# pierreaubert/math-audio

Hardware: NVIDIA B200
Metric: bem_assemble_plus_gmres_seconds_per_frequency (lower is better)
Workload: dtype f64

## Files before the change

### include/bemb200.h

```cpp
#ifndef BEMB200_H
#define BEMB200_H

#include <stdint.h>

#ifdef __cplusplus
extern "C" {
#endif

#define BEMB200_OK 0
#define BEMB200_EINVAL (-1)
#define BEMB200_ENODEVICE (-2)
#define BEMB200_ECUDA (-3)
#define BEMB200_ENOMEM (-4)
#define BEMB200_ENCCL (-5)
#define BEMB200_EUNSUPPORTED (-6)
#define BEMB200_ESINGULAR (-7)
#define BEMB200_ECALLBACK (-8)

typedef struct bemb200_ctx bemb200_ctx;
typedef struct bemb200_staged_mesh bemb200_staged_mesh;
typedef struct bemb200_matrix bemb200_matrix;

typedef struct bemb200_mesh {
    uint64_t n_nodes;
    uint64_t n_elem;
    const double* nodes;
    const uint32_t* conn;
    const uint8_t* etype;
    const double* center;
    const double* normal;
    const double* area;
    const int32_t* bc_type;
    const uint8_t* bc_len;
    const double* bc_val;
    const uint32_t* dof;
    const uint8_t* is_eval;
} bemb200_mesh;

typedef struct bemb200_physics {
    double wave_number;
    double harmonic_factor;
    double tau;
    double gamma;
} bemb200_physics;

typedef struct bemb200_gmres_info {
    uint64_t iterations;
    uint64_t restarts;
    double residual;
    int32_t converged;
} bemb200_gmres_info;

typedef struct bemb200_assembly_stats {
    uint64_t near_pairs;
    uint64_t special_pairs;
    uint64_t far_kernel_launches;
    uint64_t total_launches;
    double far_ms;
    double total_ms;
} bemb200_assembly_stats;

int bemb200_device_count(void);
int bemb200_ctx_create(int device, bemb200_ctx** out);
int bemb200_nccl_unique_id(uint8_t out[128]);
int bemb200_ctx_create_dist(int device, int rank, int nranks, const uint8_t nccl_id[128], bemb200_ctx** out);
int bemb200_ctx_create_ex(int device, int rank, int nranks, const uint8_t* nccl_id, void* cuda_stream, bemb200_ctx** out);
void bemb200_ctx_destroy(bemb200_ctx* ctx);
int bemb200_ctx_set_background(bemb200_ctx* ctx, int blocks_per_sm);
int bemb200_ctx_set_shared_gpu(bemb200_ctx* ctx, int shared);
int bemb200_matrix_boost_assembly(bemb200_matrix* m, bemb200_ctx* ctx);
int bemb200_ctx_peer_exchange_active(const bemb200_ctx* ctx, int* active);
int bemb200_matrix_set_context(bemb200_matrix* m, bemb200_ctx* ctx);
const char* bemb200_last_error(const bemb200_ctx* ctx);
void bemb200_partition(uint64_t n, int nranks, int rank, uint64_t* row_begin, uint64_t* row_end);

int bemb200_mesh_stage(bemb200_ctx* ctx, const bemb200_mesh* mesh, bemb200_staged_mesh** out);
void bemb200_staged_mesh_free(bemb200_staged_mesh* sm);
uint64_t bemb200_staged_num_dofs(const bemb200_staged_mesh* sm);
int bemb200_assemble_staged(bemb200_ctx* ctx, const bemb200_staged_mesh* sm, const bemb200_physics* phys, double beta_re,
                            double beta_im, uint64_t row_begin, uint64_t row_end, bemb200_matrix** inout);
int bemb200_assemble(bemb200_ctx* ctx, const bemb200_mesh* mesh, const bemb200_physics* phys, double beta_re,
                     double beta_im, uint64_t row_begin, uint64_t row_end, bemb200_matrix** out);
int bemb200_assembly_stats_get(const bemb200_matrix* m, bemb200_assembly_stats* out);
double bemb200_dg_dn_sign(const bemb200_staged_mesh* sm, double wave_number);

int bemb200_matrix_from_host(bemb200_ctx* ctx, const double* a_rows, uint64_t n_rows_global, uint64_t n_cols,
                             uint64_t row_begin, uint64_t row_end, bemb200_matrix** out);
void bemb200_matrix_free(bemb200_matrix* m);
uint64_t bemb200_num_rows(const bemb200_matrix* m);
uint64_t bemb200_num_cols(const bemb200_matrix* m);
uint64_t bemb200_local_row_begin(const bemb200_matrix* m);
uint64_t bemb200_local_row_end(const bemb200_matrix* m);
int bemb200_matrix_download(const bemb200_matrix* m, uint64_t row_begin, uint64_t row_end, double* out);
int bemb200_rhs_download(const bemb200_matrix* m, double* out);
int bemb200_rhs_download_full(const bemb200_matrix* m, double* out);
int bemb200_row_sum_correction(bemb200_matrix* m, double* avg);

int bemb200_apply(const bemb200_matrix* m, const double* x, double* y);
int bemb200_apply_transpose(const bemb200_matrix* m, const double* x, double* y);
int bemb200_apply_device(const bemb200_matrix* m, const double* x_dev, double* y_dev);

int bemb200_gmres(const bemb200_matrix* m, const double* b, const double* x0, uint32_t max_iterations, uint32_t restart,
                  double tolerance, double* x_out, bemb200_gmres_info* info);
int bemb200_gmres_preconditioned(const bemb200_matrix* m, const double* inv_diag, const double* b, const double* x0,
                                 uint32_t max_iterations, uint32_t restart, double tolerance, double* x_out,
                                 bemb200_gmres_info* info);
int bemb200_matrix_diagonal(const bemb200_matrix* m, double* out);
typedef struct bemb200_precond bemb200_precond;
typedef struct bemb200_precond_stats {
    uint32_t num_subdomains;
    uint32_t local_subdomains;
    uint32_t min_size, max_size;
    double avg_size;
    uint64_t inverse_bytes;
    double factor_ms;
    int32_t disjoint;
} bemb200_precond_stats;
int bemb200_schwarz_create(const bemb200_matrix* m, uint32_t num_subdomains, const uint64_t* sub_ptr, const uint64_t* sub_idx,
                           bemb200_precond** out);
void bemb200_precond_free(bemb200_precond* p);
int bemb200_precond_stats_get(const bemb200_precond* p, bemb200_precond_stats* out);
int bemb200_precond_apply(const bemb200_precond* p, const double* r, double* z);
int bemb200_gmres_schwarz(const bemb200_matrix* m, const bemb200_precond* precond, const double* b, const double* x0,
                          uint32_t max_iterations, uint32_t restart, double tolerance, double* x_out, bemb200_gmres_info* info);
typedef int (*bemb200_precond_fn)(void* user, const double* r, double* z, uint64_t n);
int bemb200_gmres_callback(const bemb200_matrix* m, bemb200_precond_fn apply, void* user, const double* b, const double* x0,
                           uint32_t max_iterations, uint32_t restart, double tolerance, double* x_out, bemb200_gmres_info* info,
                           uint64_t* precond_calls);
int bemb200_gmres_device(const bemb200_matrix* m, const double* b_dev, const double* x0_dev, uint32_t max_iterations,
                         uint32_t restart, double tolerance, double* x_dev, bemb200_gmres_info* info);
int bemb200_lu_solve(const bemb200_matrix* m, const double* b, double* x_out, int overwrite_matrix, double* factor_ms);
int bemb200_bicgstab(const bemb200_matrix* m, const double* b, uint32_t max_iterations, double tolerance, double* x_out,
                     bemb200_gmres_info* info);
int bemb200_cgs(const bemb200_matrix* m, const double* b, uint32_t max_iterations, double tolerance, double* x_out,
                bemb200_gmres_info* info);
int bemb200_gmres_batched(const bemb200_matrix* m, const double* b_all, uint32_t nrhs, uint32_t max_iterations,
                          uint32_t restart, double tolerance, double* x_all, bemb200_gmres_info* infos,
                          double* block_matvec_ms, uint64_t* block_matvecs);
int bemb200_gmres_batched_schwarz(const bemb200_matrix* m, const bemb200_precond* precond, const double* b_all, uint32_t nrhs,
                                  uint32_t max_iterations, uint32_t restart, double tolerance, double* x_all,
                                  bemb200_gmres_info* infos, double* block_matvec_ms, uint64_t* block_matvecs);
int bemb200_apply_block(const bemb200_matrix* m, const double* x_all, uint32_t nrhs, double* y_all, double* kernel_ms);
int bemb200_solver_stats(const bemb200_matrix* m, uint64_t* kernel_launches, double* matvec_ms, uint64_t* matvecs);

int bemb200_incident_rhs(const bemb200_staged_mesh* sm, const bemb200_physics* phys, double beta_re, double beta_im,
                         uint32_t n_sources, const int32_t* kinds, const double* vecs, const double* amps, double* rhs_host,
                         double* rhs_dev);
int bemb200_scattered_field(const bemb200_staged_mesh* sm, const bemb200_physics* phys, uint64_t n_eval, const double* eval_pts,
                            const double* surface_pressure, const double* surface_velocity, double* out);
int bemb200_compute_rcs(const bemb200_staged_mesh* sm, const bemb200_physics* phys, uint32_t n_dirs, const double* dirs,
                        const double* surface_pressure, double* rcs_out);

typedef struct bemb200_room_mesh bemb200_room_mesh;
int bemb200_room_mesh_stage(bemb200_ctx* ctx, const double* nodes, uint64_t n_nodes, const uint32_t* conn, uint64_t n_elem,
                            bemb200_room_mesh** out);
void bemb200_room_mesh_free(bemb200_room_mesh* rm);
uint64_t bemb200_room_mesh_num_elements(const bemb200_room_mesh* rm);
int bemb200_room_mesh_geometry(const bemb200_room_mesh* rm, double* center, double* normal, double* area);
int bemb200_room_assemble(bemb200_ctx* ctx, const bemb200_room_mesh* rm, double k, uint64_t row_begin, uint64_t row_end,
                          bemb200_matrix** inout, double* kernel_ms);
typedef struct bemb200_room_source {
    double position[3];
    double amplitude;
    const double* directivity;
    uint32_t n_horizontal, n_vertical;
} bemb200_room_source;
int bemb200_room_incident_rhs(const bemb200_room_mesh* rm, double k, uint32_t n_sources, const bemb200_room_source* sources,
                              double* rhs_host, double* rhs_dev);
int bemb200_room_field_pressure(const bemb200_room_mesh* rm, double k, uint32_t n_sources, const bemb200_room_source* sources,
                                uint64_t n_points, const double* points, const double* surface_pressure, double* out);

typedef struct bemb200_sweep bemb200_sweep;
int bemb200_sweep_create(int device, int rank, int nranks, const uint8_t* nccl_id, const bemb200_mesh* mesh, int overlap,
                         int background_blocks_per_sm, bemb200_sweep** out);
uint64_t bemb200_sweep_num_dofs(const bemb200_sweep* sw);
int bemb200_sweep_submit(bemb200_sweep* sw, const bemb200_physics* phys, double beta_re, double beta_im, const double* rhs_extra,
                         uint32_t max_iterations, uint32_t restart, double tolerance);
int bemb200_sweep_next(bemb200_sweep* sw, double* x_out, bemb200_gmres_info* info, bemb200_assembly_stats* stats, double* rhs_out);
uint64_t bemb200_sweep_boosts(const bemb200_sweep* sw);
int bemb200_sweep_set_block_jacobi(bemb200_sweep* sw, uint32_t num_subdomains, const uint64_t* sub_ptr, const uint64_t* sub_idx);
void bemb200_sweep_destroy(bemb200_sweep* sw);

typedef struct bemb200_multi bemb200_multi;
typedef struct bemb200_multi_matrix bemb200_multi_matrix;
int bemb200_multi_create(const int* devices, int n, bemb200_multi** out);
void bemb200_multi_destroy(bemb200_multi* mg);
int bemb200_multi_num_ranks(const bemb200_multi* mg);
const char* bemb200_multi_last_error(const bemb200_multi* mg);
int bemb200_multi_assemble(bemb200_multi* mg, const bemb200_mesh* mesh, const bemb200_physics* phys, double beta_re, double beta_im,
                           bemb200_multi_matrix** out);
void bemb200_multi_matrix_free(bemb200_multi_matrix* mm);
uint64_t bemb200_multi_num_rows(const bemb200_multi_matrix* mm);
int bemb200_multi_rhs_download(const bemb200_multi_matrix* mm, double* out);
int bemb200_multi_matrix_download(const bemb200_multi_matrix* mm, uint64_t row_begin, uint64_t row_end, double* out);
int bemb200_multi_gmres(const bemb200_multi_matrix* mm, const double* b, const double* x0, uint32_t max_iterations, uint32_t restart,
                        double tolerance, double* x_out, bemb200_gmres_info* info);

int bemb200_measure_fp64_peak(bemb200_ctx* ctx, double* tflops);
int bemb200_selftest_math(bemb200_ctx* ctx, uint64_t n, double xmax, double* sincos_err, double* rsqrt_relerr);
int bemb200_measure_allgather(bemb200_ctx* ctx, uint64_t bytes_per_rank, int iters, int sync_each, double* usec_per_call);
void* bemb200_matrix_device_ptr(const bemb200_matrix* m);

#ifdef __cplusplus
}
#endif
#endif
```

### include/bemb200.hpp

```cpp
#pragma once
#include <algorithm>
#include <cmath>
#include <complex>
#include <cstdint>
#include <exception>
#include <memory>
#include <stdexcept>
#include <string>
#include <utility>
#include <vector>

#include "bemb200.h"

namespace bemb200 {

using Complex64 = std::complex<double>;
static_assert(sizeof(Complex64) == 2 * sizeof(double), "std::complex<double> must be two doubles");

struct Error : std::runtime_error {
    int code;
    Error(int c, const std::string& m) : std::runtime_error("libbemb200 error " + std::to_string(c) + ": " + m), code(c) {}
};
inline void check(int rc, const bemb200_ctx* ctx = nullptr) {
    if (rc != BEMB200_OK) {
        const char* m = bemb200_last_error(ctx);
        if ((!m || !*m) && ctx) m = bemb200_last_error(nullptr);
        throw Error(rc, m ? m : "");
    }
}

struct PhysicsParams {
    double speed_of_sound, density, frequency, wave_number, omega, wave_length, harmonic_factor, pressure_factor, tau;
    PhysicsParams(double frequency_, double speed_of_sound_, double density_, bool is_internal)
        : speed_of_sound(speed_of_sound_), density(density_), frequency(frequency_) {
        const double PI = 3.14159265358979323846264338327950288;
        omega = 2.0 * PI * frequency;
        wave_number = omega / speed_of_sound;
        wave_length = speed_of_sound / frequency;
        harmonic_factor = 1.0;
        pressure_factor = density * omega * harmonic_factor;
        tau = is_internal ? -1.0 : 1.0;
    }
    double gamma() const { return 1.0; }
    Complex64 burton_miller_beta() const { return tau > 0.0 ? Complex64(0.0, harmonic_factor / wave_number) : Complex64(0.0, 0.0); }
    Complex64 burton_miller_beta_scaled(double scale) const {
        return tau > 0.0 ? Complex64(0.0, harmonic_factor * scale / wave_number) : Complex64(0.0, 0.0);
    }
    Complex64 burton_miller_beta_optimal(double element_size) const {
        return tau > 0.0 ? Complex64(0.0, harmonic_factor / (wave_number + 1.0 / element_size)) : Complex64(0.0, 0.0);
    }
    std::pair<Complex64, double> burton_miller_beta_adaptive(double radius) const {
        if (tau <= 0.0) return {Complex64(0.0, 0.0), 1.0};
        const double ka = wave_number * radius;
        const double scale = ka < 0.5 ? 1.0 : (ka < 1.2 ? 4.0 : (ka < 1.8 ? 8.0 : 16.0));
        return {Complex64(0.0, harmonic_factor * scale / wave_number), scale};
    }
};

enum class ElementType { Tri3, Quad4 };
enum class ElementProperty { Surface = 0, MidFace = 1, Evaluation = 2 };

struct BoundaryCondition {
    enum Kind { Velocity, Pressure, VelocityWithAdmittance, TransferAdmittance, TransferWithSurfaceAdmittance } kind = Velocity;
    std::vector<Complex64> values{Complex64(0.0, 0.0)};
    static BoundaryCondition velocity(std::vector<Complex64> v) { return {Velocity, std::move(v)}; }
    static BoundaryCondition pressure(std::vector<Complex64> p) { return {Pressure, std::move(p)}; }
};

struct Element {
    std::vector<std::size_t> connectivity;
    ElementType element_type = ElementType::Tri3;
    ElementProperty property = ElementProperty::Surface;
    double normal[3] = {0, 0, 0};
    double center[3] = {0, 0, 0};
    double area = 0.0;
    BoundaryCondition boundary_condition;
    std::size_t group = 0;
    std::vector<std::size_t> dof_addresses;
};

class Context {
public:
    explicit Context(int device = 0) { check(bemb200_ctx_create(device, &h_)); }
    Context(int device, int rank, int nranks, const uint8_t* nccl_id, void* cuda_stream = nullptr) {
        check(bemb200_ctx_create_ex(device, rank, nranks, nccl_id, cuda_stream, &h_));
    }
    ~Context() { bemb200_ctx_destroy(h_); }
    Context(const Context&) = delete;
    Context& operator=(const Context&) = delete;
    bemb200_ctx* handle() const { return h_; }
    void set_background(int blocks_per_sm) { check(bemb200_ctx_set_background(h_, blocks_per_sm), h_); }
    void set_shared_gpu(bool shared) { check(bemb200_ctx_set_shared_gpu(h_, shared ? 1 : 0), h_); }
    bool peer_exchange_active() const {
        int a = 0;
        check(bemb200_ctx_peer_exchange_active(h_, &a), h_);
        return a != 0;
    }

private:
    bemb200_ctx* h_ = nullptr;
};

struct LinearOperator {
    virtual ~LinearOperator() = default;
    virtual std::size_t num_rows() const = 0;
    virtual std::size_t num_cols() const = 0;
    virtual std::vector<Complex64> apply(const std::vector<Complex64>& x) const = 0;
    virtual std::vector<Complex64> apply_transpose(const std::vector<Complex64>& x) const = 0;
    virtual std::vector<Complex64> apply_hermitian(const std::vector<Complex64>& x) const {
        std::vector<Complex64> xc(x.size());
        for (std::size_t i = 0; i < x.size(); ++i) xc[i] = std::conj(x[i]);
        std::vector<Complex64> y = apply_transpose(xc);
        for (auto& v : y) v = std::conj(v);
        return y;
    }
    bool is_square() const { return num_rows() == num_cols(); }
};

class DenseOperator : public LinearOperator {
public:
    DenseOperator(const Context& ctx, const std::vector<Complex64>& matrix, std::size_t n_rows, std::size_t n_cols) : ctx_(&ctx) {
        if (matrix.size() != n_rows * n_cols) throw std::invalid_argument("DenseOperator: matrix size does not match its shape");
        check(bemb200_matrix_from_host(ctx.handle(), reinterpret_cast<const double*>(matrix.data()), n_rows, n_cols, 0, n_rows, &m_),
              ctx.handle());
    }
    DenseOperator(const Context& ctx, bemb200_matrix* owned) : ctx_(&ctx), m_(owned) {}
    ~DenseOperator() override { bemb200_matrix_free(m_); }
    DenseOperator(const DenseOperator&) = delete;
    DenseOperator& operator=(const DenseOperator&) = delete;
    std::size_t num_rows() const override { return bemb200_num_rows(m_); }
    std::size_t num_cols() const override { return bemb200_num_cols(m_); }
    std::vector<Complex64> apply(const std::vector<Complex64>& x) const override {
        if (x.size() != num_cols()) throw std::invalid_argument("apply: vector length does not match num_cols");
        std::vector<Complex64> y(num_rows());
        check(bemb200_apply(m_, reinterpret_cast<const double*>(x.data()), reinterpret_cast<double*>(y.data())), ctx_->handle());
        return y;
    }
    std::vector<Complex64> apply_transpose(const std::vector<Complex64>& x) const override {
        if (x.size() != num_rows()) throw std::invalid_argument("apply_transpose: vector length does not match num_rows");
        std::vector<Complex64> y(num_cols());
        check(bemb200_apply_transpose(m_, reinterpret_cast<const double*>(x.data()), reinterpret_cast<double*>(y.data())),
              ctx_->handle());
        return y;
    }
    std::vector<Complex64> rows(std::size_t row_begin, std::size_t row_end) const {
        std::vector<Complex64> out((row_end - row_begin) * num_cols());
        check(bemb200_matrix_download(m_, row_begin, row_end, reinterpret_cast<double*>(out.data())), ctx_->handle());
        return out;
    }
    std::vector<Complex64> diagonal() const {
        std::vector<Complex64> d(num_rows());
        check(bemb200_matrix_diagonal(m_, reinterpret_cast<double*>(d.data())), ctx_->handle());
        return d;
    }
    bemb200_matrix* handle() const { return m_; }
    const Context& context() const { return *ctx_; }

private:
    const Context* ctx_;
    bemb200_matrix* m_ = nullptr;
};

struct TbemSystem {
    std::unique_ptr<DenseOperator> matrix;
    std::vector<Complex64> rhs;
    std::size_t num_dofs = 0;
};

struct MeshSoA {
    std::vector<uint32_t> conn, dof;
    std::vector<uint8_t> etype, bc_len, is_eval;
    std::vector<double> center, normal, area, bc_val;
    std::vector<int32_t> bc_type;
    std::size_t n_elem = 0, ndof = 0;
    MeshSoA(const std::vector<Element>& elements) {
        const std::size_t n = elements.size();
        n_elem = n;
        conn.assign(4 * n, 0xFFFFFFFFu); dof.assign(n, 0);
        etype.resize(n); bc_len.assign(n, 1); is_eval.assign(n, 0);
        center.resize(3 * n); normal.resize(3 * n); area.resize(n); bc_val.assign(8 * n, 0.0);
        bc_type.assign(n, 0);
        for (std::size_t i = 0; i < n; ++i) {
            const Element& e = elements[i];
            etype[i] = e.element_type == ElementType::Tri3 ? 3 : 4;
            if (e.connectivity.size() != etype[i]) throw std::invalid_argument("element connectivity does not match its type");
            for (std::size_t v = 0; v < e.connectivity.size(); ++v) conn[4 * i + v] = static_cast<uint32_t>(e.connectivity[v]);
            for (int d = 0; d < 3; ++d) { center[3 * i + d] = e.center[d]; normal[3 * i + d] = e.normal[d]; }
            area[i] = e.area;
            const BoundaryCondition& bc = e.boundary_condition;
            std::vector<Complex64> vals;
            switch (bc.kind) {
                case BoundaryCondition::Velocity: case BoundaryCondition::VelocityWithAdmittance: bc_type[i] = 0; vals = bc.values; break;
                case BoundaryCondition::Pressure: bc_type[i] = 1; vals = bc.values; break;
                default: bc_type[i] = 2; vals = {Complex64(0.0, 0.0)}; break;
            }
            if (vals.empty() || vals.size() > 4) throw std::invalid_argument("boundary condition needs 1..4 values");
            bc_len[i] = static_cast<uint8_t>(vals.size());
            for (std::size_t k = 0; k < vals.size(); ++k) { bc_val[8 * i + 2 * k] = vals[k].real(); bc_val[8 * i + 2 * k + 1] = vals[k].imag(); }
            is_eval[i] = e.property == ElementProperty::Evaluation;
            if (!is_eval[i]) {
                if (e.dof_addresses.empty()) throw std::invalid_argument("boundary element without dof address");
                dof[i] = static_cast<uint32_t>(e.dof_addresses[0]);
                ++ndof;
            }
        }
    }
    bemb200_mesh view(const std::vector<double>& nodes) const {
        return bemb200_mesh{nodes.size() / 3, n_elem, nodes.data(), conn.data(), etype.data(), center.data(), normal.data(), area.data(),
                            bc_type.data(), bc_len.data(), bc_val.data(), dof.data(), is_eval.data()};
    }
};
inline bemb200_physics physics_abi(const PhysicsParams& p) { return bemb200_physics{p.wave_number, p.harmonic_factor, p.tau, p.gamma()}; }

inline TbemSystem tbem_system_from_handle(const Context& ctx, bemb200_matrix* m, std::size_t ndof) {
    TbemSystem sys;
    sys.matrix = std::make_unique<DenseOperator>(ctx, m);
    sys.num_dofs = ndof;
    sys.rhs.resize(ndof);
    check(bemb200_rhs_download_full(m, reinterpret_cast<double*>(sys.rhs.data())), ctx.handle());
    return sys;
}

inline TbemSystem build_tbem_system_with_beta(const Context& ctx, const std::vector<Element>& elements,
                                              const std::vector<double>& nodes, const PhysicsParams& physics, Complex64 beta) {
    const MeshSoA soa(elements);
    const bemb200_mesh mesh = soa.view(nodes);
    const bemb200_physics phys = physics_abi(physics);
    bemb200_matrix* m = nullptr;
    check(bemb200_assemble(ctx.handle(), &mesh, &phys, beta.real(), beta.imag(), 0, soa.ndof, &m), ctx.handle());
    return tbem_system_from_handle(ctx, m, soa.ndof);
}

class StagedMesh {
public:
    StagedMesh(const Context& ctx, const std::vector<Element>& elements, const std::vector<double>& nodes) : ctx_(&ctx) {
        const MeshSoA soa(elements);
        const bemb200_mesh mesh = soa.view(nodes);
        check(bemb200_mesh_stage(ctx.handle(), &mesh, &h_), ctx.handle());
        num_dofs_ = soa.ndof;
        bool sequential = true;
        std::vector<uint32_t> map;
        std::vector<uint8_t> seen(soa.ndof, 0);
        bool permutation = true;
        for (std::size_t i = 0; i < soa.n_elem; ++i) {
            if (soa.is_eval[i]) continue;
            const uint32_t d = soa.dof[i];
            sequential = sequential && d == map.size();
            if (d >= soa.ndof || seen[d]) permutation = false; else seen[d] = 1;
            map.push_back(d);
        }
        if (!sequential && permutation) enum_to_dof_ = std::move(map);
    }
    std::vector<Complex64> in_dof_order(const std::vector<Complex64>& values) const {
        if (enum_to_dof_.empty()) return values;
        std::vector<Complex64> out(values.size());
        for (std::size_t j = 0; j < values.size(); ++j) out[enum_to_dof_[j]] = values[j];
        return out;
    }
    ~StagedMesh() { bemb200_staged_mesh_free(h_); }
    StagedMesh(const StagedMesh&) = delete;
    StagedMesh& operator=(const StagedMesh&) = delete;
    bemb200_staged_mesh* handle() const { return h_; }
    const Context& context() const { return *ctx_; }
    std::size_t num_dofs() const { return num_dofs_; }
    double dg_dn_sign(double wave_number) const { return bemb200_dg_dn_sign(h_, wave_number); }

private:
    const Context* ctx_;
    bemb200_staged_mesh* h_ = nullptr;
    std::size_t num_dofs_ = 0;
    std::vector<uint32_t> enum_to_dof_;
};
inline TbemSystem build_tbem_system_with_beta(const StagedMesh& mesh, const PhysicsParams& physics, Complex64 beta) {
    const bemb200_physics phys = physics_abi(physics);
    bemb200_matrix* m = nullptr;
    check(bemb200_assemble_staged(mesh.context().handle(), mesh.handle(), &phys, beta.real(), beta.imag(), 0, mesh.num_dofs(), &m),
          mesh.context().handle());
    return tbem_system_from_handle(mesh.context(), m, mesh.num_dofs());
}
inline TbemSystem build_tbem_system(const Context& ctx, const std::vector<Element>& el, const std::vector<double>& nodes,
                                    const PhysicsParams& ph) {
    return build_tbem_system_with_beta(ctx, el, nodes, ph, ph.burton_miller_beta());
}
inline TbemSystem build_tbem_system_scaled(const Context& ctx, const std::vector<Element>& el, const std::vector<double>& nodes,
                                           const PhysicsParams& ph, double scale) {
    return build_tbem_system_with_beta(ctx, el, nodes, ph, ph.burton_miller_beta_scaled(scale));
}
inline TbemSystem build_tbem_system_bounded(const Context& ctx, const std::vector<Element>& el, const std::vector<double>& nodes,
                                            const PhysicsParams& ph, double avg_element_size) {
    return build_tbem_system_with_beta(ctx, el, nodes, ph, ph.burton_miller_beta_optimal(avg_element_size));
}
inline double apply_row_sum_correction(TbemSystem& system) {
    double avg = 0.0;
    check(bemb200_row_sum_correction(system.matrix->handle(), &avg), system.matrix->context().handle());
    return avg;
}

inline std::pair<TbemSystem, double> build_tbem_system_corrected(const Context& ctx, const std::vector<Element>& el,
                                                                 const std::vector<double>& nodes, const PhysicsParams& ph) {
    TbemSystem system = build_tbem_system(ctx, el, nodes, ph);
    const double avg = apply_row_sum_correction(system);
    return {std::move(system), avg};
}

struct GmresConfig {
    std::size_t max_iterations = 100;
    std::size_t restart = 30;
    double tolerance = 1e-6;
    std::size_t print_interval = 0;
};
struct GmresSolution {
    std::vector<Complex64> x;
    std::size_t iterations = 0, restarts = 0;
    double residual = 0.0;
    bool converged = false;
};
inline GmresSolution gmres_with_guess(const DenseOperator& op, const std::vector<Complex64>& b, const std::vector<Complex64>* x0,
                                      const GmresConfig& config) {
    if (b.size() != op.num_rows() || (x0 && x0->size() != b.size())) throw std::invalid_argument("gmres: vector lengths must match");
    GmresSolution s;
    s.x.resize(b.size());
    bemb200_gmres_info info{};
    check(bemb200_gmres(op.handle(), reinterpret_cast<const double*>(b.data()), x0 ? reinterpret_cast<const double*>(x0->data()) : nullptr,
                        static_cast<uint32_t>(config.max_iterations), static_cast<uint32_t>(config.restart), config.tolerance,
                        reinterpret_cast<double*>(s.x.data()), &info),
          op.context().handle());
    s.iterations = info.iterations; s.restarts = info.restarts; s.residual = info.residual; s.converged = info.converged != 0;
    return s;
}
inline GmresSolution gmres(const DenseOperator& op, const std::vector<Complex64>& b, const GmresConfig& config) {
    return gmres_with_guess(op, b, nullptr, config);
}
inline GmresSolution solve_gmres(const DenseOperator& op, const std::vector<Complex64>& b, const GmresConfig& config) {
    return gmres(op, b, config);
}

struct IdentityPreconditioner {};
struct DiagonalPreconditioner {
    std::vector<Complex64> inv_diag;
    static DiagonalPreconditioner from_diagonal(const std::vector<Complex64>& diag) {
        DiagonalPreconditioner p;
        p.inv_diag.resize(diag.size());
        for (std::size_t i = 0; i < diag.size(); ++i) {
            const double re = diag[i].real(), im = diag[i].imag(), ns = re * re + im * im;
            p.inv_diag[i] = std::hypot(re, im) > 1e-30 ? Complex64(re / ns, -im / ns) : Complex64(1.0, 0.0);
        }
        return p;
    }
};
inline GmresSolution gmres_preconditioned_impl(const DenseOperator& op, const std::vector<Complex64>* inv_diag,
                                               const std::vector<Complex64>& b, const std::vector<Complex64>* x0,
                                               const GmresConfig& config) {
    if (b.size() != op.num_rows() || (x0 && x0->size() != b.size()) || (inv_diag && inv_diag->size() != b.size()))
        throw std::invalid_argument("gmres_preconditioned: vector lengths must match");
    GmresSolution s;
    s.x.resize(b.size());
    bemb200_gmres_info info{};
    check(bemb200_gmres_preconditioned(op.handle(), inv_diag ? reinterpret_cast<const double*>(inv_diag->data()) : nullptr,
                                       reinterpret_cast<const double*>(b.data()),
                                       x0 ? reinterpret_cast<const double*>(x0->data()) : nullptr,
                                       static_cast<uint32_t>(config.max_iterations), static_cast<uint32_t>(config.restart),
                                       config.tolerance, reinterpret_cast<double*>(s.x.data()), &info),
          op.context().handle());
    s.iterations = info.iterations; s.restarts = info.restarts; s.residual = info.residual; s.converged = info.converged != 0;
    return s;
}
inline GmresSolution gmres_preconditioned(const DenseOperator& op, const IdentityPreconditioner&, const std::vector<Complex64>& b,
                                          const GmresConfig& config) {
    return gmres_preconditioned_impl(op, nullptr, b, nullptr, config);
}
inline GmresSolution gmres_preconditioned(const DenseOperator& op, const DiagonalPreconditioner& p, const std::vector<Complex64>& b,
                                          const GmresConfig& config) {
    return gmres_preconditioned_impl(op, &p.inv_diag, b, nullptr, config);
}
inline GmresSolution gmres_preconditioned_with_guess(const DenseOperator& op, const DiagonalPreconditioner& p,
                                                     const std::vector<Complex64>& b, const std::vector<Complex64>* x0,
                                                     const GmresConfig& config) {
    return gmres_preconditioned_impl(op, &p.inv_diag, b, x0, config);
}

class AdditiveSchwarzPreconditioner {
public:
    static AdditiveSchwarzPreconditioner from_operator(const DenseOperator& op, std::size_t num_subdomains) {
        AdditiveSchwarzPreconditioner p(op);
        check(bemb200_schwarz_create(op.handle(), static_cast<uint32_t>(num_subdomains), nullptr, nullptr, &p.h_), op.context().handle());
        return p;
    }
    static AdditiveSchwarzPreconditioner from_subdomains(const DenseOperator& op, const std::vector<std::vector<uint64_t>>& subdomains) {
        AdditiveSchwarzPreconditioner p(op);
        std::vector<uint64_t> ptr(1, 0), idx;
        for (const auto& sd : subdomains) {
            idx.insert(idx.end(), sd.begin(), sd.end());
            ptr.push_back(idx.size());
        }
        check(bemb200_schwarz_create(op.handle(), static_cast<uint32_t>(subdomains.size()), ptr.data(), idx.empty() ? ptr.data() : idx.data(),
// ... 433 lines not shown
```

### math_audio_b200/_capi.py

```python
from __future__ import annotations

import ctypes as C
from pathlib import Path

import numpy as np

_HERE = Path(__file__).resolve().parent
LIB_PATH = _HERE / "lib" / "libbemb200.so"

OK = 0
ERRORS = {-1: "EINVAL", -2: "ENODEVICE", -3: "ECUDA", -4: "ENOMEM", -5: "ENCCL", -6: "EUNSUPPORTED", -7: "ESINGULAR", -8: "ECALLBACK"}


class Bemb200Error(RuntimeError):
    def __init__(self, code: int, msg: str):
        super().__init__(f"libbemb200 {ERRORS.get(code, code)}: {msg}")
        self.code = code


class CMesh(C.Structure):
    _fields_ = [
        ("n_nodes", C.c_uint64), ("n_elem", C.c_uint64),
        ("nodes", C.c_void_p), ("conn", C.c_void_p), ("etype", C.c_void_p),
        ("center", C.c_void_p), ("normal", C.c_void_p), ("area", C.c_void_p),
        ("bc_type", C.c_void_p), ("bc_len", C.c_void_p), ("bc_val", C.c_void_p),
        ("dof", C.c_void_p), ("is_eval", C.c_void_p),
    ]


class CPhysics(C.Structure):
    _fields_ = [("wave_number", C.c_double), ("harmonic_factor", C.c_double), ("tau", C.c_double), ("gamma", C.c_double)]


class CGmresInfo(C.Structure):
    _fields_ = [("iterations", C.c_uint64), ("restarts", C.c_uint64), ("residual", C.c_double), ("converged", C.c_int32)]


class CAssemblyStats(C.Structure):
    _fields_ = [("near_pairs", C.c_uint64), ("special_pairs", C.c_uint64), ("far_kernel_launches", C.c_uint64),
                ("total_launches", C.c_uint64), ("far_ms", C.c_double), ("total_ms", C.c_double)]


class CPrecondStats(C.Structure):
    _fields_ = [("num_subdomains", C.c_uint32), ("local_subdomains", C.c_uint32), ("min_size", C.c_uint32), ("max_size", C.c_uint32),
                ("avg_size", C.c_double), ("inverse_bytes", C.c_uint64), ("factor_ms", C.c_double), ("disjoint", C.c_int32)]


class CRoomSource(C.Structure):
    _fields_ = [("position", C.c_double * 3), ("amplitude", C.c_double), ("directivity", C.c_void_p),
                ("n_horizontal", C.c_uint32), ("n_vertical", C.c_uint32)]


_VP = C.c_void_p
_PP = C.POINTER(C.c_void_p)
PRECOND_FN = C.CFUNCTYPE(C.c_int, C.c_void_p, C.POINTER(C.c_double), C.POINTER(C.c_double), C.c_uint64)

SYMBOLS = {
    "bemb200_device_count": (C.c_int, []),
    "bemb200_ctx_create": (C.c_int, [C.c_int, _PP]),
    "bemb200_nccl_unique_id": (C.c_int, [_VP]),
    "bemb200_ctx_create_dist": (C.c_int, [C.c_int, C.c_int, C.c_int, _VP, _PP]),
    "bemb200_ctx_create_ex": (C.c_int, [C.c_int, C.c_int, C.c_int, _VP, _VP, _PP]),
    "bemb200_ctx_destroy": (None, [_VP]),
    "bemb200_matrix_set_context": (C.c_int, [_VP, _VP]),
    "bemb200_ctx_set_background": (C.c_int, [_VP, C.c_int]),
    "bemb200_ctx_set_shared_gpu": (C.c_int, [_VP, C.c_int]),
    "bemb200_matrix_boost_assembly": (C.c_int, [_VP, _VP]),
    "bemb200_ctx_peer_exchange_active": (C.c_int, [_VP, C.POINTER(C.c_int)]),
    "bemb200_last_error": (C.c_char_p, [_VP]),
    "bemb200_partition": (None, [C.c_uint64, C.c_int, C.c_int, C.POINTER(C.c_uint64), C.POINTER(C.c_uint64)]),
    "bemb200_mesh_stage": (C.c_int, [_VP, C.POINTER(CMesh), _PP]),
    "bemb200_staged_mesh_free": (None, [_VP]),
    "bemb200_staged_num_dofs": (C.c_uint64, [_VP]),
    "bemb200_assemble_staged": (C.c_int, [_VP, _VP, C.POINTER(CPhysics), C.c_double, C.c_double, C.c_uint64, C.c_uint64, _PP]),
    "bemb200_assemble": (C.c_int, [_VP, C.POINTER(CMesh), C.POINTER(CPhysics), C.c_double, C.c_double, C.c_uint64, C.c_uint64, _PP]),
    "bemb200_assembly_stats_get": (C.c_int, [_VP, C.POINTER(CAssemblyStats)]),
    "bemb200_dg_dn_sign": (C.c_double, [_VP, C.c_double]),
    "bemb200_matrix_from_host": (C.c_int, [_VP, _VP, C.c_uint64, C.c_uint64, C.c_uint64, C.c_uint64, _PP]),
    "bemb200_matrix_free": (None, [_VP]),
    "bemb200_num_rows": (C.c_uint64, [_VP]),
    "bemb200_num_cols": (C.c_uint64, [_VP]),
    "bemb200_local_row_begin": (C.c_uint64, [_VP]),
    "bemb200_local_row_end": (C.c_uint64, [_VP]),
    "bemb200_matrix_download": (C.c_int, [_VP, C.c_uint64, C.c_uint64, _VP]),
    "bemb200_rhs_download": (C.c_int, [_VP, _VP]),
    "bemb200_rhs_download_full": (C.c_int, [_VP, _VP]),
    "bemb200_row_sum_correction": (C.c_int, [_VP, C.POINTER(C.c_double)]),
    "bemb200_apply": (C.c_int, [_VP, _VP, _VP]),
    "bemb200_apply_transpose": (C.c_int, [_VP, _VP, _VP]),
    "bemb200_apply_device": (C.c_int, [_VP, _VP, _VP]),
    "bemb200_gmres": (C.c_int, [_VP, _VP, _VP, C.c_uint32, C.c_uint32, C.c_double, _VP, C.POINTER(CGmresInfo)]),
    "bemb200_gmres_preconditioned": (C.c_int, [_VP, _VP, _VP, _VP, C.c_uint32, C.c_uint32, C.c_double, _VP, C.POINTER(CGmresInfo)]),
    "bemb200_matrix_diagonal": (C.c_int, [_VP, _VP]),
    "bemb200_schwarz_create": (C.c_int, [_VP, C.c_uint32, _VP, _VP, _PP]),
    "bemb200_precond_free": (None, [_VP]),
    "bemb200_precond_stats_get": (C.c_int, [_VP, C.POINTER(CPrecondStats)]),
    "bemb200_precond_apply": (C.c_int, [_VP, _VP, _VP]),
    "bemb200_gmres_schwarz": (C.c_int, [_VP, _VP, _VP, _VP, C.c_uint32, C.c_uint32, C.c_double, _VP, C.POINTER(CGmresInfo)]),
    "bemb200_gmres_callback": (C.c_int, [_VP, PRECOND_FN, _VP, _VP, _VP, C.c_uint32, C.c_uint32, C.c_double, _VP, C.POINTER(CGmresInfo),
                                         C.POINTER(C.c_uint64)]),
    "bemb200_gmres_device": (C.c_int, [_VP, _VP, _VP, C.c_uint32, C.c_uint32, C.c_double, _VP, C.POINTER(CGmresInfo)]),
    "bemb200_gmres_batched": (C.c_int, [_VP, _VP, C.c_uint32, C.c_uint32, C.c_uint32, C.c_double, _VP, C.POINTER(CGmresInfo),
                                        C.POINTER(C.c_double), C.POINTER(C.c_uint64)]),
    "bemb200_gmres_batched_schwarz": (C.c_int, [_VP, _VP, _VP, C.c_uint32, C.c_uint32, C.c_uint32, C.c_double, _VP, C.POINTER(CGmresInfo),
                                                C.POINTER(C.c_double), C.POINTER(C.c_uint64)]),
    "bemb200_apply_block": (C.c_int, [_VP, _VP, C.c_uint32, _VP, C.POINTER(C.c_double)]),
    "bemb200_solver_stats": (C.c_int, [_VP, C.POINTER(C.c_uint64), C.POINTER(C.c_double), C.POINTER(C.c_uint64)]),
    "bemb200_incident_rhs": (C.c_int, [_VP, C.POINTER(CPhysics), C.c_double, C.c_double, C.c_uint32, _VP, _VP, _VP, _VP, _VP]),
    "bemb200_scattered_field": (C.c_int, [_VP, C.POINTER(CPhysics), C.c_uint64, _VP, _VP, _VP, _VP]),
    "bemb200_compute_rcs": (C.c_int, [_VP, C.POINTER(CPhysics), C.c_uint32, _VP, _VP, _VP]),
    "bemb200_bicgstab": (C.c_int, [_VP, _VP, C.c_uint32, C.c_double, _VP, C.POINTER(CGmresInfo)]),
    "bemb200_cgs": (C.c_int, [_VP, _VP, C.c_uint32, C.c_double, _VP, C.POINTER(CGmresInfo)]),
    "bemb200_lu_solve": (C.c_int, [_VP, _VP, _VP, C.c_int, C.POINTER(C.c_double)]),
    "bemb200_room_mesh_stage": (C.c_int, [_VP, _VP, C.c_uint64, _VP, C.c_uint64, _PP]),
    "bemb200_room_mesh_free": (None, [_VP]),
    "bemb200_room_mesh_num_elements": (C.c_uint64, [_VP]),
    "bemb200_room_mesh_geometry": (C.c_int, [_VP, _VP, _VP, _VP]),
    "bemb200_room_assemble": (C.c_int, [_VP, _VP, C.c_double, C.c_uint64, C.c_uint64, _PP, C.POINTER(C.c_double)]),
    "bemb200_room_incident_rhs": (C.c_int, [_VP, C.c_double, C.c_uint32, C.POINTER(CRoomSource), _VP, _VP]),
    "bemb200_room_field_pressure": (C.c_int, [_VP, C.c_double, C.c_uint32, C.POINTER(CRoomSource), C.c_uint64, _VP, _VP, _VP]),
    "bemb200_measure_fp64_peak": (C.c_int, [_VP, C.POINTER(C.c_double)]),
    "bemb200_selftest_math": (C.c_int, [_VP, C.c_uint64, C.c_double, C.POINTER(C.c_double), C.POINTER(C.c_double)]),
    "bemb200_measure_allgather": (C.c_int, [_VP, C.c_uint64, C.c_int, C.c_int, C.POINTER(C.c_double)]),
    "bemb200_matrix_device_ptr": (_VP, [_VP]),
    "bemb200_sweep_create": (C.c_int, [C.c_int, C.c_int, C.c_int, _VP, C.POINTER(CMesh), C.c_int, C.c_int, _PP]),
    "bemb200_sweep_num_dofs": (C.c_uint64, [_VP]),
    "bemb200_sweep_submit": (C.c_int, [_VP, C.POINTER(CPhysics), C.c_double, C.c_double, _VP, C.c_uint32, C.c_uint32, C.c_double]),
    "bemb200_sweep_next": (C.c_int, [_VP, _VP, C.POINTER(CGmresInfo), C.POINTER(CAssemblyStats), _VP]),
    "bemb200_sweep_boosts": (C.c_uint64, [_VP]),
    "bemb200_sweep_set_block_jacobi": (C.c_int, [_VP, C.c_uint32, _VP, _VP]),
    "bemb200_sweep_destroy": (None, [_VP]),
    "bemb200_multi_create": (C.c_int, [C.POINTER(C.c_int), C.c_int, _PP]),
    "bemb200_multi_destroy": (None, [_VP]),
    "bemb200_multi_num_ranks": (C.c_int, [_VP]),
    "bemb200_multi_last_error": (C.c_char_p, [_VP]),
    "bemb200_multi_assemble": (C.c_int, [_VP, C.POINTER(CMesh), C.POINTER(CPhysics), C.c_double, C.c_double, _PP]),
    "bemb200_multi_matrix_free": (None, [_VP]),
    "bemb200_multi_num_rows": (C.c_uint64, [_VP]),
    "bemb200_multi_rhs_download": (C.c_int, [_VP, _VP]),
    "bemb200_multi_matrix_download": (C.c_int, [_VP, C.c_uint64, C.c_uint64, _VP]),
    "bemb200_multi_gmres": (C.c_int, [_VP, _VP, _VP, C.c_uint32, C.c_uint32, C.c_double, _VP, C.POINTER(CGmresInfo)]),
}

_lib = None


def lib():
    global _lib
    if _lib is None:
        if not LIB_PATH.exists():
            raise FileNotFoundError(
                f"{LIB_PATH} not found: build it with `python -m math_audio_b200.build` (nvcc, sm_100a). "
                "There is no CPU fallback.")
        l = C.CDLL(str(LIB_PATH))
        for name, (res, args) in SYMBOLS.items():
            fn = getattr(l, name)
            fn.restype = res
            fn.argtypes = args
        _lib = l
    return _lib


def check(rc: int, ctx=None):
    if rc != OK:
        msg = lib().bemb200_last_error(ctx)
        if (not msg) and ctx is not None:
            msg = lib().bemb200_last_error(None)
        raise Bemb200Error(rc, (msg or b"").decode(errors="replace"))


def ptr(a: np.ndarray):
    return a.ctypes.data_as(C.c_void_p)


def cmesh(mesh) -> CMesh:
    arrs = dict(
        nodes=np.ascontiguousarray(mesh.nodes, dtype=np.float64),
        conn=np.ascontiguousarray(mesh.conn, dtype=np.uint32),
        etype=np.ascontiguousarray(mesh.etype, dtype=np.uint8),
        center=np.ascontiguousarray(mesh.center, dtype=np.float64),
        normal=np.ascontiguousarray(mesh.normal, dtype=np.float64),
        area=np.ascontiguousarray(mesh.area, dtype=np.float64),
        bc_type=np.ascontiguousarray(mesh.bc_type, dtype=np.int32),
        bc_len=np.ascontiguousarray(mesh.bc_len, dtype=np.uint8),
        bc_val=np.ascontiguousarray(mesh.bc_val, dtype=np.complex128),
        dof=np.ascontiguousarray(mesh.dof, dtype=np.uint32),
        is_eval=np.ascontiguousarray(mesh.is_eval, dtype=np.uint8),
    )
    m = CMesh(mesh.n_nodes, mesh.n_elem, *[ptr(arrs[k]) for k in
              ("nodes", "conn", "etype", "center", "normal", "area", "bc_type", "bc_len", "bc_val", "dof", "is_eval")])
    m._keep = arrs
    return m


def mesh_nbytes(mesh) -> int:
    return int(sum(getattr(mesh, k).nbytes for k in
                   ("nodes", "conn", "etype", "center", "normal", "area", "bc_type", "bc_len", "bc_val", "dof", "is_eval")))
```

### math_audio_b200/bem.py

```python
from __future__ import annotations

import ctypes as C
from dataclasses import dataclass
from typing import List, Optional, Sequence

import numpy as np

from . import _capi
from .mesh import Mesh
from .types import PhysicsParams


class Context:

    def __init__(self, device: int = 0, rank: int = 0, nranks: int = 1, nccl_id: Optional[bytes] = None,
                 cuda_stream: int = 0):
        self._lib = _capi.lib()
        self._h = C.c_void_p()
        idp = None
        if nranks > 1 and nccl_id is not None:
            assert len(nccl_id) == 128
            self._idbuf = (C.c_uint8 * 128).from_buffer_copy(nccl_id)
            idp = C.cast(self._idbuf, C.c_void_p)
        _capi.check(self._lib.bemb200_ctx_create_ex(device, rank, nranks, idp, C.c_void_p(cuda_stream or None), C.byref(self._h)))
        self.device, self.rank, self.nranks = device, rank, nranks

    @staticmethod
    def nccl_unique_id() -> bytes:
        buf = (C.c_uint8 * 128)()
        _capi.check(_capi.lib().bemb200_nccl_unique_id(C.cast(buf, C.c_void_p)))
        return bytes(buf)

    def partition(self, n: int):
        b, e = C.c_uint64(), C.c_uint64()
        self._lib.bemb200_partition(n, self.nranks, self.rank, C.byref(b), C.byref(e))
        return int(b.value), int(e.value)

    def measure_fp64_peak(self) -> float:
        t = C.c_double()
        _capi.check(self._lib.bemb200_measure_fp64_peak(self._h, C.byref(t)), self._h)
        return float(t.value)

    def selftest_math(self, n: int = 1 << 22, xmax: float = 200.0):
        a, b = C.c_double(), C.c_double()
        _capi.check(self._lib.bemb200_selftest_math(self._h, n, xmax, C.byref(a), C.byref(b)), self._h)
        return float(a.value), float(b.value)

    def set_background(self, blocks_per_sm: int) -> None:
        _capi.check(self._lib.bemb200_ctx_set_background(self._h, blocks_per_sm), self._h)

    def peer_exchange_active(self) -> bool:
        a = C.c_int(0)
        _capi.check(self._lib.bemb200_ctx_peer_exchange_active(self._h, C.byref(a)), self._h)
        return bool(a.value)

    def set_shared_gpu(self, shared: bool) -> None:
        _capi.check(self._lib.bemb200_ctx_set_shared_gpu(self._h, 1 if shared else 0), self._h)

    def measure_allgather(self, bytes_per_rank: int, iters: int = 200, sync_each: bool = False) -> float:
        t = C.c_double()
        _capi.check(self._lib.bemb200_measure_allgather(self._h, bytes_per_rank, iters, 1 if sync_each else 0, C.byref(t)), self._h)
        return float(t.value)

    def close(self):
        if self._h:
            self._lib.bemb200_ctx_destroy(self._h)
            self._h = C.c_void_p()

    def __del__(self):
        try:
            self.close()
        except Exception:
            pass


_default_ctx: Optional[Context] = None


class MultiGpu:

    def __init__(self, devices):
        self._lib = _capi.lib()
        self._h = C.c_void_p()
        arr = (C.c_int * len(devices))(*[int(d) for d in devices])
        _capi.check(self._lib.bemb200_multi_create(arr, len(devices), C.byref(self._h)), None)
        self.nranks = len(devices)

    def build_tbem_system_with_beta(self, mesh: Mesh, physics: PhysicsParams, beta: complex) -> "MultiSystem":
        cm = _capi.cmesh(mesh)
        ph = _cphys(physics)
        beta = complex(beta)
        h = C.c_void_p()
        _capi.check(self._lib.bemb200_multi_assemble(self._h, C.byref(cm), C.byref(ph), beta.real, beta.imag, C.byref(h)), None)
        return MultiSystem(self, h)

    def close(self):
        if self._h:
            self._lib.bemb200_multi_destroy(self._h)
            self._h = C.c_void_p()

    def __del__(self):
        try:
            self.close()
        except Exception:
            pass


class MultiSystem:

    def __init__(self, group: MultiGpu, handle):
        self.group, self._h, self._lib = group, handle, _capi.lib()
        self.num_dofs = int(self._lib.bemb200_multi_num_rows(self._h))

    @property
    def rhs(self) -> np.ndarray:
        out = np.empty(self.num_dofs, dtype=np.complex128)
        _capi.check(self._lib.bemb200_multi_rhs_download(self._h, _capi.ptr(out)), None)
        return out

    def rows(self, row_begin: int = 0, row_end: Optional[int] = None) -> np.ndarray:
        row_end = self.num_dofs if row_end is None else row_end
        out = np.empty((row_end - row_begin, self.num_dofs), dtype=np.complex128)
        _capi.check(self._lib.bemb200_multi_matrix_download(self._h, row_begin, row_end, _capi.ptr(out)), None)
        return out

    def gmres(self, b: np.ndarray, config: "GmresConfig", x0: Optional[np.ndarray] = None) -> "GmresSolution":
        b = np.ascontiguousarray(b, dtype=np.complex128)
        if b.shape != (self.num_dofs,):
            raise ValueError("gmres: b has the wrong length")
        x0a = np.ascontiguousarray(x0, dtype=np.complex128) if x0 is not None else None
        x = np.empty(self.num_dofs, dtype=np.complex128)
        info = _capi.CGmresInfo()
        _capi.check(self._lib.bemb200_multi_gmres(self._h, _capi.ptr(b), _capi.ptr(x0a) if x0a is not None else None,
                                                  config.max_iterations, config.restart, config.tolerance, _capi.ptr(x), C.byref(info)), None)
        return GmresSolution(x=x, iterations=int(info.iterations), restarts=int(info.restarts), residual=float(info.residual),
                             converged=bool(info.converged))

    def close(self):
        if self._h:
            self._lib.bemb200_multi_matrix_free(self._h)
            self._h = C.c_void_p()

    def __del__(self):
        try:
            self.close()
        except Exception:
            pass


def default_context() -> Context:
    global _default_ctx
    if _default_ctx is None:
        _default_ctx = Context(0)
    return _default_ctx


def enumeration_to_dof(mesh: Mesh) -> Optional[np.ndarray]:
    dof = np.asarray(mesh.dof, dtype=np.int64)[np.asarray(mesh.is_eval) == 0]
    if np.array_equal(dof, np.arange(dof.size)):
        return None
    if not np.array_equal(np.sort(dof), np.arange(dof.size)):
        return None
    return dof


def surface_values_in_dof_order(enum_to_dof: Optional[np.ndarray], values: np.ndarray) -> np.ndarray:
    if enum_to_dof is None:
        return values
    out = np.empty_like(values)
    out[enum_to_dof] = values
    return out


class StagedMesh:

    def __init__(self, mesh: Mesh, ctx: Optional[Context] = None):
        self.ctx = ctx or default_context()
        self._lib = _capi.lib()
        self._h = C.c_void_p()
        cm = _capi.cmesh(mesh)
        _capi.check(self._lib.bemb200_mesh_stage(self.ctx._h, C.byref(cm), C.byref(self._h)), self.ctx._h)
        self.num_dofs = int(self._lib.bemb200_staged_num_dofs(self._h))
        self.nbytes_host = _capi.mesh_nbytes(mesh)
        self.enum_to_dof = enumeration_to_dof(mesh)

    def dg_dn_sign(self, wave_number: float) -> float:
        return float(self._lib.bemb200_dg_dn_sign(self._h, wave_number))

    def close(self):
        if self._h:
            self._lib.bemb200_staged_mesh_free(self._h)
            self._h = C.c_void_p()

    def __del__(self):
        try:
            self.close()
        except Exception:
            pass


def _cphys(physics: PhysicsParams) -> _capi.CPhysics:
    return _capi.CPhysics(physics.wave_number, physics.harmonic_factor, physics.tau, physics.gamma())


class DeviceMatrix:

    def __init__(self, ctx: Context, handle: C.c_void_p):
        self.ctx = ctx
        self._lib = _capi.lib()
        self._h = handle

    @property
    def shape(self):
        return int(self._lib.bemb200_num_rows(self._h)), int(self._lib.bemb200_num_cols(self._h))

    @property
    def local_rows(self):
        return int(self._lib.bemb200_local_row_begin(self._h)), int(self._lib.bemb200_local_row_end(self._h))

    def rows(self, row_begin: Optional[int] = None, row_end: Optional[int] = None) -> np.ndarray:
        lb, le = self.local_rows
        row_begin = lb if row_begin is None else row_begin
        row_end = le if row_end is None else row_end
        out = np.empty((row_end - row_begin, self.shape[1]), dtype=np.complex128)
        _capi.check(self._lib.bemb200_matrix_download(self._h, row_begin, row_end, _capi.ptr(out)), self.ctx._h)
        return out

    def rhs(self) -> np.ndarray:
        lb, le = self.local_rows
        out = np.empty(le - lb, dtype=np.complex128)
        _capi.check(self._lib.bemb200_rhs_download(self._h, _capi.ptr(out)), self.ctx._h)
        return out

    def assembly_stats(self) -> dict:
        st = _capi.CAssemblyStats()
        _capi.check(self._lib.bemb200_assembly_stats_get(self._h, C.byref(st)), self.ctx._h)
        return {k: getattr(st, k) for k, _ in st._fields_}

    def solver_stats(self) -> dict:
        a, b, c = C.c_uint64(), C.c_double(), C.c_uint64()
        _capi.check(self._lib.bemb200_solver_stats(self._h, C.byref(a), C.byref(b), C.byref(c)), self.ctx._h)
        return dict(kernel_launches=int(a.value), matvec_ms=float(b.value), matvecs=int(c.value))

    def device_ptr(self) -> int:
        return int(self._lib.bemb200_matrix_device_ptr(self._h) or 0)

    def boost_assembly(self, ctx: "Context") -> None:
        _capi.check(self._lib.bemb200_matrix_boost_assembly(self._h, ctx._h), ctx._h)

    def set_context(self, ctx: "Context") -> None:
        _capi.check(self._lib.bemb200_matrix_set_context(self._h, ctx._h), ctx._h)
        self.ctx = ctx

    def close(self):
        if self._h:
            self._lib.bemb200_matrix_free(self._h)
            self._h = C.c_void_p()

    def __del__(self):
        try:
            self.close()
        except Exception:
            pass


@dataclass
class TbemSystem:

    matrix: DeviceMatrix
    rhs: Optional[np.ndarray]
    num_dofs: int

    def rhs_full(self, n: Optional[int] = None) -> np.ndarray:
        out = np.empty(self.num_dofs, dtype=np.complex128)
        _capi.check(_capi.lib().bemb200_rhs_download_full(self.matrix._h, _capi.ptr(out)), self.matrix.ctx._h)
        return out


def build_tbem_system_with_beta(elements: Mesh | StagedMesh, physics: PhysicsParams, beta: complex,
                                ctx: Optional[Context] = None, rows=None, reuse: Optional[TbemSystem] = None,
                                fetch_rhs: bool = True) -> TbemSystem:
    lib = _capi.lib()
    staged = elements if isinstance(elements, StagedMesh) else StagedMesh(elements, ctx)
    ctx = staged.ctx
    n = staged.num_dofs
    r0, r1 = rows if rows is not None else ctx.partition(n)
    h = reuse.matrix._h if reuse is not None else C.c_void_p()
    ph = _cphys(physics)
    beta = complex(beta)
    _capi.check(lib.bemb200_assemble_staged(ctx._h, staged._h, C.byref(ph), beta.real, beta.imag, r0, r1, C.byref(h)), ctx._h)
    mat = reuse.matrix if reuse is not None else DeviceMatrix(ctx, h)
    return TbemSystem(matrix=mat, rhs=mat.rhs() if fetch_rhs else None, num_dofs=n)


def build_tbem_system(elements, physics: PhysicsParams, **kw) -> TbemSystem:
    return build_tbem_system_with_beta(elements, physics, physics.burton_miller_beta(), **kw)


def build_tbem_system_scaled(elements, physics: PhysicsParams, scale: float, **kw) -> TbemSystem:
    return build_tbem_system_with_beta(elements, physics, physics.burton_miller_beta_scaled(scale), **kw)


def build_tbem_system_bounded(elements, physics: PhysicsParams, avg_element_size: float, **kw) -> TbemSystem:
    return build_tbem_system_with_beta(elements, physics, physics.burton_miller_beta_optimal(avg_element_size), **kw)


def apply_row_sum_correction(system: TbemSystem) -> float:
    avg = C.c_double()
    _capi.check(_capi.lib().bemb200_row_sum_correction(system.matrix._h, C.byref(avg)), system.matrix.ctx._h)
    return float(avg.value)


def build_tbem_system_corrected(elements, physics: PhysicsParams, **kw):
    system = build_tbem_system(elements, physics, **kw)
    return system, apply_row_sum_correction(system)


class DenseOperator:

    def __init__(self, matrix, ctx: Optional[Context] = None):
        if isinstance(matrix, TbemSystem):
            matrix = matrix.matrix
        if isinstance(matrix, DeviceMatrix):
            self.matrix = matrix
        else:
            a = np.ascontiguousarray(matrix, dtype=np.complex128)
            if a.ndim != 2:
                raise ValueError("DenseOperator needs a 2-D matrix")
            ctx = ctx or default_context()
            r0, r1 = ctx.partition(a.shape[0])
            h = C.c_void_p()
            loc = np.ascontiguousarray(a[r0:r1])
            _capi.check(_capi.lib().bemb200_matrix_from_host(ctx._h, _capi.ptr(loc), a.shape[0], a.shape[1], r0, r1, C.byref(h)), ctx._h)
            self.matrix = DeviceMatrix(ctx, h)
        self._lib = _capi.lib()

    def num_rows(self) -> int:
        return self.matrix.shape[0]

    def num_cols(self) -> int:
        return self.matrix.shape[1]

    def is_square(self) -> bool:
        return self.num_rows() == self.num_cols()

    def apply(self, x: np.ndarray) -> np.ndarray:
        x = np.ascontiguousarray(x, dtype=np.complex128)
        if x.shape != (self.num_cols(),):
            raise ValueError(f"apply: x has shape {x.shape}, operator has {self.num_cols()} columns")
        y = np.empty(self.num_rows(), dtype=np.complex128)
        _capi.check(self._lib.bemb200_apply(self.matrix._h, _capi.ptr(x), _capi.ptr(y)), self.matrix.ctx._h)
        return y
# ... 555 lines not shown
```

### math_audio_b200/csrc/api.cu

```cuda
#include <cmath>
#include <cstdio>
#include <cstring>
#include <dlfcn.h>

#include "api_internal.h"

using namespace bemb;

namespace {
std::string g_last_error;
std::mutex g_err_mu;
}

namespace bemb {
int set_error(bemb200_ctx* ctx, int code, const std::string& msg) {
    {
        std::lock_guard<std::mutex> lk(g_err_mu);
        g_last_error = msg;
    }
    if (ctx) ctx->err = msg;
    return code;
}
int cuda_fail(bemb200_ctx* ctx, cudaError_t e, const char* what) {
    cudaGetLastError();
    return set_error(ctx, e == cudaErrorMemoryAllocation ? BEMB200_ENOMEM : BEMB200_ECUDA,
                     std::string("CUDA error '") + cudaGetErrorString(e) + "' in " + what);
}
}

namespace ncclshim {
typedef struct { char internal[128]; } UniqueId;
typedef int (*GetUniqueId_t)(UniqueId*);
typedef int (*CommInitRank_t)(void**, int, UniqueId, int);
typedef int (*CommDestroy_t)(void*);
typedef int (*AllGather_t)(const void*, void*, size_t, int, void*, cudaStream_t);
typedef const char* (*GetErrorString_t)(int);
void* handle = nullptr;
GetUniqueId_t GetUniqueId = nullptr;
CommInitRank_t CommInitRank = nullptr;
CommDestroy_t CommDestroy = nullptr;
AllGather_t AllGather = nullptr;
GetErrorString_t GetErrorString = nullptr;
bool load(std::string& why) {
    if (handle) return true;
    const char* names[] = {"libnccl.so.2", "libnccl.so"};
    for (const char* n : names) {
        handle = dlopen(n, RTLD_NOW | RTLD_GLOBAL);
        if (handle) break;
    }
    if (!handle) {
        why = std::string("cannot dlopen libnccl.so.2: ") + dlerror();
        return false;
    }
    GetUniqueId = (GetUniqueId_t)dlsym(handle, "ncclGetUniqueId");
    CommInitRank = (CommInitRank_t)dlsym(handle, "ncclCommInitRank");
    CommDestroy = (CommDestroy_t)dlsym(handle, "ncclCommDestroy");
    AllGather = (AllGather_t)dlsym(handle, "ncclAllGather");
    GetErrorString = (GetErrorString_t)dlsym(handle, "ncclGetErrorString");
    if (!GetUniqueId || !CommInitRank || !CommDestroy || !AllGather) {
        why = "libnccl is missing required symbols";
        return false;
    }
    return true;
}
}

namespace bemb {
int nccl_allgather_bytes(bemb200_ctx* ctx, const void* send, void* recv, size_t count_bytes) {
    if (ctx->nranks == 1) return BEMB200_OK;
    if (!ctx->nccl_comm) return set_error(ctx, BEMB200_ENCCL, "this context was created without a communicator (assembly only)");
    int rc = ncclshim::AllGather(send, recv, count_bytes, 0, ctx->nccl_comm, ctx->stream);
    if (rc != 0)
        return set_error(ctx, BEMB200_ENCCL, std::string("ncclAllGather failed: ") +
                                                 (ncclshim::GetErrorString ? ncclshim::GetErrorString(rc) : "?"));
    return BEMB200_OK;
}
}

template <class T>
static int dev_alloc_copy(bemb200_staged_mesh* sm, T** dst, const std::vector<T>& src) {
    size_t bytes = src.size() * sizeof(T);
    if (bytes == 0) bytes = sizeof(T);
    BEMB_CUDA(sm->ctx, cudaMallocAsync((void**)dst, bytes, sm->ctx->stream));
    sm->allocs.push_back(*dst);
    if (!src.empty()) BEMB_CUDA(sm->ctx, cudaMemcpyAsync(*dst, src.data(), src.size() * sizeof(T), cudaMemcpyHostToDevice, sm->ctx->stream));
    return BEMB200_OK;
}
template <class T>
static int dev_alloc(bemb200_staged_mesh* sm, T** dst, size_t count) {
    BEMB_CUDA(sm->ctx, cudaMallocAsync((void**)dst, (count ? count : 1) * sizeof(T), sm->ctx->stream));
    sm->allocs.push_back(*dst);
    return BEMB200_OK;
}

extern "C" {

int bemb200_device_count(void) {
    int n = 0;
    if (cudaGetDeviceCount(&n) != cudaSuccess) {
        cudaGetLastError();
        return 0;
    }
    return n;
}

static int ctx_create_common(int device, void* ext_stream, bemb200_ctx** out) {
    if (!out) return set_error(nullptr, BEMB200_EINVAL, "out is NULL");
    *out = nullptr;
    int n = bemb200_device_count();
    if (n <= 0) return set_error(nullptr, BEMB200_ENODEVICE, "no CUDA device visible (libbemb200 has no CPU fallback)");
    if (device < 0 || device >= n) return set_error(nullptr, BEMB200_EINVAL, "device index out of range");
    bemb200_ctx* c = new bemb200_ctx();
    c->device = device;
    BEMB_CUDA(c, cudaSetDevice(device));
    cudaDeviceProp prop;
    BEMB_CUDA(c, cudaGetDeviceProperties(&prop, device));
    if (prop.major != 10) {
        std::string msg = std::string("device '") + prop.name + "' is not sm_100 (libbemb200 ships sm_100a code only)";
        delete c;
        return set_error(nullptr, BEMB200_EUNSUPPORTED, msg);
    }
    {
        cudaMemPool_t pool;
        if (cudaDeviceGetDefaultMemPool(&pool, device) == cudaSuccess) {
            unsigned long long thr = ~0ull;
            cudaMemPoolSetAttribute(pool, cudaMemPoolAttrReleaseThreshold, &thr);
        }
        cudaGetLastError();
    }
    if (ext_stream) {
        c->stream = (cudaStream_t)ext_stream;
        c->own_stream = false;
    } else {
        BEMB_CUDA(c, cudaStreamCreateWithFlags(&c->stream, cudaStreamNonBlocking));
    }
    *out = c;
    return BEMB200_OK;
}

int bemb200_ctx_create(int device, bemb200_ctx** out) { return ctx_create_common(device, nullptr, out); }

int bemb200_nccl_unique_id(uint8_t out[128]) {
    std::string why;
    if (!ncclshim::load(why)) return set_error(nullptr, BEMB200_ENCCL, why);
    ncclshim::UniqueId id;
    int rc = ncclshim::GetUniqueId(&id);
    if (rc != 0) return set_error(nullptr, BEMB200_ENCCL, "ncclGetUniqueId failed");
    std::memcpy(out, id.internal, 128);
    return BEMB200_OK;
}

int bemb200_ctx_create_dist(int device, int rank, int nranks, const uint8_t nccl_id[128], bemb200_ctx** out) {
    return bemb200_ctx_create_ex(device, rank, nranks, nccl_id, nullptr, out);
}

int bemb200_ctx_create_ex(int device, int rank, int nranks, const uint8_t* nccl_id, void* cuda_stream, bemb200_ctx** out) {
    if (nranks < 1 || rank < 0 || rank >= nranks) return set_error(nullptr, BEMB200_EINVAL, "bad rank/nranks");
    int rc = ctx_create_common(device, cuda_stream, out);
    if (rc != BEMB200_OK) return rc;
    bemb200_ctx* c = *out;
    c->rank = rank;
    c->nranks = nranks;
    if (nranks > 1 && nccl_id) {
        std::string why;
        if (!ncclshim::load(why)) {
            bemb200_ctx_destroy(c);
            *out = nullptr;
            return set_error(nullptr, BEMB200_ENCCL, why);
        }
        ncclshim::UniqueId id;
        std::memcpy(id.internal, nccl_id, 128);
        int nrc = ncclshim::CommInitRank(&c->nccl_comm, nranks, id, rank);
        if (nrc != 0) {
            bemb200_ctx_destroy(c);
            *out = nullptr;
            return set_error(nullptr, BEMB200_ENCCL, "ncclCommInitRank failed");
        }
    }
    return BEMB200_OK;
}

void bemb200_ctx_destroy(bemb200_ctx* ctx) {
    if (!ctx) return;
    cudaSetDevice(ctx->device);
    free_peer_exchange(ctx, false);
    if (ctx->nccl_comm && ncclshim::CommDestroy) ncclshim::CommDestroy(ctx->nccl_comm);
    if (ctx->stream && ctx->own_stream) cudaStreamDestroy(ctx->stream);
    delete ctx;
}

const char* bemb200_last_error(const bemb200_ctx* ctx) {
    if (ctx) return ctx->err.c_str();
    return g_last_error.c_str();
}

void bemb200_partition(uint64_t n, int nranks, int rank, uint64_t* row_begin, uint64_t* row_end) {
    uint64_t chunk = (n + (uint64_t)nranks - 1) / (uint64_t)nranks;
    uint64_t b = chunk * (uint64_t)rank, e = b + chunk;
    if (b > n) b = n;
    if (e > n) e = n;
    *row_begin = b;
    *row_end = e;
}

void bemb200_staged_mesh_free(bemb200_staged_mesh* sm) {
    if (!sm) return;
    cudaSetDevice(sm->ctx->device);
    for (void* p : sm->allocs) cudaFreeAsync(p, sm->ctx->stream);
    delete sm;
}

uint64_t bemb200_staged_num_dofs(const bemb200_staged_mesh* sm) { return sm ? sm->dm.n : 0; }

int bemb200_mesh_stage(bemb200_ctx* ctx, const bemb200_mesh* mesh, bemb200_staged_mesh** out) {
    if (!ctx) return set_error(nullptr, BEMB200_EINVAL, "ctx is NULL");
    if (!mesh || !out) return set_error(ctx, BEMB200_EINVAL, "mesh/out is NULL");
    *out = nullptr;
    std::lock_guard<std::mutex> lk(ctx->mu);
    BEMB_CUDA(ctx, cudaSetDevice(ctx->device));
    const uint64_t ne = mesh->n_elem;
    uint64_t ndof = 0;
    for (uint64_t e = 0; e < ne; ++e) ndof += mesh->is_eval[e] ? 0 : 1;
    if (ndof == 0) return set_error(ctx, BEMB200_EINVAL, "mesh has no boundary (non-evaluation) element");
    if (ndof > 0x7fffffffull) return set_error(ctx, BEMB200_EINVAL, "too many DOFs");
    std::vector<int64_t> elem_of_dof(ndof, -1);
    for (uint64_t e = 0; e < ne; ++e) {
        if (mesh->is_eval[e]) continue;
        uint64_t d = mesh->dof[e];
        if (d >= ndof || elem_of_dof[d] != -1)
            return set_error(ctx, BEMB200_EINVAL, "dof addresses of boundary elements must be a permutation of 0..ndof-1");
        elem_of_dof[d] = (int64_t)e;
        int et = mesh->etype[e];
        if (et != 3 && et != 4) return set_error(ctx, BEMB200_EINVAL, "etype must be 3 (Tri3) or 4 (Quad4)");
        for (int v = 0; v < et; ++v)
            if (mesh->conn[4 * e + v] >= mesh->n_nodes) return set_error(ctx, BEMB200_EINVAL, "connectivity index out of range");
        if (mesh->bc_len[e] < 1 || mesh->bc_len[e] > 4) return set_error(ctx, BEMB200_EINVAL, "bc_len must be 1..4");
    }
    bemb200_staged_mesh* sm = new bemb200_staged_mesh();
    sm->ctx = ctx;
    DeviceMesh& dm = sm->dm;
    dm.n = (uint32_t)ndof;
    dm.ntiles = (uint32_t)((ndof + TILE - 1) / TILE);
    std::vector<double> coords(ndof * 12, 0.0), area(ndof), src(ndof * 8, 0.0);
    std::vector<uint8_t> etype(ndof), bclen(ndof), nz(ndof);
    std::vector<int32_t> bctype(ndof);
    std::vector<cplx> bcval(ndof * 4);
    for (uint64_t d = 0; d < ndof; ++d) {
        const uint64_t e = (uint64_t)elem_of_dof[d];
        const int et = mesh->etype[e];
        etype[d] = (uint8_t)et;
        for (int v = 0; v < et; ++v)
            for (int c = 0; c < 3; ++c) coords[12 * d + 3 * v + c] = mesh->nodes[3 * (uint64_t)mesh->conn[4 * e + v] + c];
        area[d] = mesh->area[e];
        for (int c = 0; c < 3; ++c) {
            src[8 * d + c] = mesh->center[3 * e + c];
            src[8 * d + 3 + c] = mesh->normal[3 * e + c];
        }
        bctype[d] = mesh->bc_type[e];
        bclen[d] = mesh->bc_len[e];
        bool nonzero = false;
        for (int i = 0; i < 4; ++i) {
            cplx v = C(0, 0);
            if (i < mesh->bc_len[e]) v = C(mesh->bc_val[8 * e + 2 * i], mesh->bc_val[8 * e + 2 * i + 1]);
            bcval[4 * d + i] = v;
            if (i < mesh->bc_len[e] && std::hypot(v.re, v.im) > 1e-15) nonzero = true;
        }
        nz[d] = nonzero ? 1 : 0;
    }
    {
        double avg = 0.0;
        uint64_t n_calc = ne < 100 ? ne : 100;
        for (uint64_t e = 0; e < n_calc; ++e) {
            const double* c = mesh->center + 3 * e;
            double s = 0.0;
            s = s + c[0] * c[0];
            s = s + c[1] * c[1];
            s = s + c[2] * c[2];
            avg += std::sqrt(s);
        }
        if (n_calc > 0) avg /= (double)n_calc;
        dm.avg_radius_first100 = avg;
    }
    int rc;
#define STAGE_TRY(x)                         \
    do {                                     \
        rc = (x);                            \
        if (rc != BEMB200_OK) {              \
            bemb200_staged_mesh_free(sm);    \
            return rc;                       \
        }                                    \
    } while (0)
    STAGE_TRY(dev_alloc_copy(sm, &dm.coords, coords));
    STAGE_TRY(dev_alloc_copy(sm, &dm.etype, etype));
    STAGE_TRY(dev_alloc_copy(sm, &dm.area, area));
    STAGE_TRY(dev_alloc_copy(sm, &dm.src, src));
    STAGE_TRY(dev_alloc_copy(sm, &dm.bc_type, bctype));
    STAGE_TRY(dev_alloc_copy(sm, &dm.bc_len, bclen));
    STAGE_TRY(dev_alloc_copy(sm, &dm.bc_val, bcval));
    STAGE_TRY(dev_alloc_copy(sm, &dm.nonzero_bc, nz));
    STAGE_TRY(dev_alloc(sm, &dm.esize, ndof));
    STAGE_TRY(dev_alloc(sm, &dm.far_k, (size_t)dm.ntiles * NQ_MAX * TILE));
    STAGE_TRY(dev_alloc(sm, &dm.far_c, (size_t)dm.ntiles * FAR_NCONST * TILE));
    STAGE_TRY(dev_alloc(sm, &dm.col_class, (size_t)dm.ntiles * TILE));
    cudaError_t e = launch_prep(dm, ctx->stream);
    if (e != cudaSuccess) {
        bemb200_staged_mesh_free(sm);
        return cuda_fail(ctx, e, "prep_kernel launch");
    }
    std::vector<uint8_t> cls((size_t)dm.ntiles * TILE);
    e = cudaMemcpyAsync(cls.data(), dm.col_class, cls.size(), cudaMemcpyDeviceToHost, ctx->stream);
    if (e == cudaSuccess) e = cudaStreamSynchronize(ctx->stream);
    if (e != cudaSuccess) {
        bemb200_staged_mesh_free(sm);
        return cuda_fail(ctx, e, "prep_kernel");
    }
    std::vector<uint32_t> special, rhs_tri, rhs_quad;
    for (uint32_t j = 0; j < dm.n; ++j) {
        if (cls[j] == COL_SPECIAL) special.push_back(j);
        else if (cls[j] == COL_FLAT_TRI) { dm.n_flat_tri++; if (nz[j]) rhs_tri.push_back(j); }
        else if (cls[j] == COL_FLAT_QUAD) { dm.n_flat_quad++; if (nz[j]) rhs_quad.push_back(j); }
    }
    dm.n_special = (uint32_t)special.size();
    dm.n_rhs_tri = (uint32_t)rhs_tri.size();
    dm.n_rhs_quad = (uint32_t)rhs_quad.size();
    STAGE_TRY(dev_alloc_copy(sm, &dm.special_cols, special));
    STAGE_TRY(dev_alloc_copy(sm, &dm.rhs_cols_tri, rhs_tri));
    STAGE_TRY(dev_alloc_copy(sm, &dm.rhs_cols_quad, rhs_quad));
    e = cudaStreamSynchronize(ctx->stream);
    if (e != cudaSuccess) {
        bemb200_staged_mesh_free(sm);
        return cuda_fail(ctx, e, "stage sync");
    }
#undef STAGE_TRY
    *out = sm;
    return BEMB200_OK;
}

double bemb200_dg_dn_sign(const bemb200_staged_mesh* sm, double wave_number) {
    if (!sm) return 0.0;
    double ka = wave_number * sm->dm.avg_radius_first100;
    return ka < 0.5 ? 1.0 : -1.0;
}

static int matrix_alloc(bemb200_ctx* ctx, uint64_t n_rows, uint64_t n_cols, uint64_t r0, uint64_t r1, bool with_near,
                        bemb200_matrix** out) {
    bemb200_matrix* m = new bemb200_matrix();
    m->ctx = ctx;
    m->n_rows = n_rows;
    m->n_cols = n_cols;
    m->r0 = r0;
    m->r1 = r1;
    const uint64_t nloc = r1 - r0;
    cudaError_t e = cudaMalloc((void**)&m->A, (nloc * n_cols + 1) * sizeof(cplx));
    if (e == cudaSuccess) e = cudaMalloc((void**)&m->rhs, (nloc + 1) * sizeof(cplx));
    if (e == cudaSuccess) e = cudaMemsetAsync(m->rhs, 0, (nloc + 1) * sizeof(cplx), ctx->stream);
    if (e == cudaSuccess && with_near) {
        m->near_cap = (unsigned int)(nloc * 64 + 4096);
        e = cudaMalloc((void**)&m->near_list, (size_t)m->near_cap * sizeof(uint2));
        if (e == cudaSuccess) e = cudaMalloc((void**)&m->near_count, sizeof(unsigned int));
        if (e == cudaSuccess) e = cudaMalloc((void**)&m->work_counters, 2 * sizeof(unsigned int));
        if (e == cudaSuccess) e = cudaEventCreateWithFlags(&m->far_ready_ev, cudaEventDisableTiming);
        if (e == cudaSuccess) e = cudaEventCreateWithFlags(&m->boost_ev, cudaEventDisableTiming);
    }
    for (int i = 0; i < 4 && e == cudaSuccess; ++i) e = cudaEventCreate(&m->ev[i]);
    if (e != cudaSuccess) {
        bemb200_matrix_free(m);
        return cuda_fail(ctx, e, "matrix allocation");
    }
    *out = m;
    return BEMB200_OK;
}

}
namespace bemb {
int matrix_alloc_plain(bemb200_ctx* ctx, uint64_t n_rows, uint64_t n_cols, uint64_t r0, uint64_t r1, bemb200_matrix** out) {
    return matrix_alloc(ctx, n_rows, n_cols, r0, r1, false, out);
}
}
extern "C" {

void bemb200_matrix_free(bemb200_matrix* m) {
    if (!m) return;
    cudaSetDevice(m->ctx->device);
    free_workspace(m);
    if (m->A) cudaFree(m->A);
    if (m->rhs) cudaFree(m->rhs);
    if (m->near_list) cudaFree(m->near_list);
    if (m->near_count) cudaFree(m->near_count);
    if (m->work_counters) cudaFree(m->work_counters);
    if (m->far_ready_ev) cudaEventDestroy(m->far_ready_ev);
    if (m->boost_ev) cudaEventDestroy(m->boost_ev);
    for (int i = 0; i < 4; ++i)
        if (m->ev[i]) cudaEventDestroy(m->ev[i]);
    delete m;
}

int bemb200_assemble_staged(bemb200_ctx* ctx, const bemb200_staged_mesh* sm, const bemb200_physics* phys, double beta_re,
                            double beta_im, uint64_t row_begin, uint64_t row_end, bemb200_matrix** inout) {
    if (!ctx) return set_error(nullptr, BEMB200_EINVAL, "ctx is NULL");
    if (!sm || !phys || !inout) return set_error(ctx, BEMB200_EINVAL, "NULL argument");
    const DeviceMesh& dm = sm->dm;
    if (row_begin > row_end || row_end > dm.n) return set_error(ctx, BEMB200_EINVAL, "row range outside [0, num_dofs]");
    if (!(phys->wave_number > 0.0)) return set_error(ctx, BEMB200_EINVAL, "wave_number must be > 0");
    std::lock_guard<std::mutex> lk(ctx->mu);
    BEMB_CUDA(ctx, cudaSetDevice(ctx->device));
    bemb200_matrix* m = *inout;
    if (m) {
        if (m->n_rows != dm.n || m->n_cols != dm.n || m->r0 != row_begin || m->r1 != row_end || !m->near_list)
            return set_error(ctx, BEMB200_EINVAL, "matrix handle to reuse has a different shape / row range");
    } else {
        int rc = matrix_alloc(ctx, dm.n, dm.n, row_begin, row_end, true, &m);
        if (rc != BEMB200_OK) return rc;
    }
    Phys ph;
    ph.k = phys->wave_number;
    ph.wavruim = phys->harmonic_factor * phys->wave_number;
    ph.k2 = phys->wave_number * phys->wave_number;
    ph.tau = phys->tau;
    ph.gamma = phys->gamma;
    ph.sign = bemb200_dg_dn_sign(sm, phys->wave_number);
    ph.beta = C(beta_re, beta_im);
    ph.beta_unscaled = phys->tau > 0.0 ? C(0.0, phys->harmonic_factor / phys->wave_number) : C(0.0, 0.0);
    const uint64_t nloc = row_end - row_begin;
    cudaStream_t s = ctx->stream;
    int rc = BEMB200_OK;
    unsigned int count = 0;
    auto fail = [&](int code) {
        if (!*inout) bemb200_matrix_free(m);
        return code;
    };
#define ASM_CUDA(call)                                                 \
    do {                                                               \
        cudaError_t _e = (call);                                       \
        if (_e != cudaSuccess) return fail(cuda_fail(ctx, _e, #call)); \
    } while (0)
    ASM_CUDA(cudaMemsetAsync(m->rhs, 0, (nloc + 1) * sizeof(cplx), s));
    if (dm.n_special) ASM_CUDA(cudaMemsetAsync(m->A, 0, nloc * dm.n * sizeof(cplx), s));
    ASM_CUDA(cudaEventRecord(m->ev[0], s));
    for (int attempt = 0; attempt < 2; ++attempt) {
        ASM_CUDA(cudaMemsetAsync(m->near_count, 0, sizeof(unsigned int), s));
        const int bg = ctx->background_blocks_per_sm.load();
        const bool boostable = bg > 0 && attempt == 0 && m->work_counters;
        if (boostable) {
            ASM_CUDA(cudaMemsetAsync(m->work_counters, 0, 2 * sizeof(unsigned int), s));
            ASM_CUDA(cudaEventRecord(m->far_ready_ev, s));
        }
        ASM_CUDA(cudaEventRecord(m->ev[1], s));
        {
            std::lock_guard<std::mutex> bl(m->boost_mu);
            m->relaunch.clear();
            m->boost_pending = false;
            cudaError_t fe = launch_far(dm, ph, row_begin, row_end, m->A, dm.n, m->near_list, m->near_cap, m->near_count, bg,
                                        boostable ? m->work_counters : nullptr, boostable ? &m->relaunch : nullptr, s);
            if (fe != cudaSuccess) return fail(cuda_fail(ctx, fe, "launch_far"));
            m->far_running = boostable;
        }
        ASM_CUDA(cudaEventRecord(m->ev[2], s));
        ASM_CUDA(cudaMemcpyAsync(&count, m->near_count, sizeof(unsigned int), cudaMemcpyDeviceToHost, s));
        ASM_CUDA(cudaStreamSynchronize(s));
        {
            bool pending;
            {
                std::lock_guard<std::mutex> bl(m->boost_mu);
                m->far_running = false;
                pending = m->boost_pending;
                m->boost_pending = false;
                m->relaunch.clear();
            }
            if (pending) {
                ASM_CUDA(cudaEventSynchronize(m->boost_ev));
                ASM_CUDA(cudaMemcpyAsync(&count, m->near_count, sizeof(unsigned int), cudaMemcpyDeviceToHost, s));
                ASM_CUDA(cudaStreamSynchronize(s));
            }
        }
        if (count <= m->near_cap) break;
        cudaFree(m->near_list);
        m->near_list = nullptr;
        m->near_cap = count + 1024;
        ASM_CUDA(cudaMalloc((void**)&m->near_list, (size_t)m->near_cap * sizeof(uint2)));
    }
    if (count > m->near_cap) {
        if (!*inout) bemb200_matrix_free(m);
        return set_error(ctx, BEMB200_ENOMEM, "near-field pair list overflowed twice (pathological mesh: more near pairs than the list can hold)");
    }
    ASM_CUDA(launch_near_list(dm, ph, row_begin, m->A, dm.n, m->rhs, m->near_list, count, s));
    ASM_CUDA(launch_rhs_far(dm, ph, row_begin, row_end, m->rhs, s));
    ASM_CUDA(launch_special(dm, ph, row_begin, row_end, m->A, dm.n, m->rhs, s));
    ASM_CUDA(launch_self(dm, ph, row_begin, row_end, m->A, dm.n, m->rhs, s));
    ASM_CUDA(cudaEventRecord(m->ev[3], s));
    ASM_CUDA(cudaStreamSynchronize(s));
#undef ASM_CUDA
    float far_ms = 0.f, tot_ms = 0.f;
    cudaEventElapsedTime(&far_ms, m->ev[1], m->ev[2]);
    cudaEventElapsedTime(&tot_ms, m->ev[0], m->ev[3]);
    m->stats.near_pairs = count;
    m->stats.special_pairs = (uint64_t)dm.n_special * nloc;
    m->stats.far_kernel_launches = (uint64_t)far_kernel_launch_count(dm);
    m->stats.total_launches = m->stats.far_kernel_launches + (count ? 1 : 0) + (dm.n_special ? 1 : 0) + 1 +
                              (dm.n_rhs_tri ? 1 : 0) + (dm.n_rhs_quad ? 1 : 0);
    m->stats.far_ms = far_ms;
    m->stats.total_ms = tot_ms;
    *inout = m;
    return rc;
}

int bemb200_assemble(bemb200_ctx* ctx, const bemb200_mesh* mesh, const bemb200_physics* phys, double beta_re,
                     double beta_im, uint64_t row_begin, uint64_t row_end, bemb200_matrix** out) {
    if (!out) return set_error(ctx, BEMB200_EINVAL, "out is NULL");
    *out = nullptr;
    bemb200_staged_mesh* sm = nullptr;
    int rc = bemb200_mesh_stage(ctx, mesh, &sm);
    if (rc != BEMB200_OK) return rc;
    rc = bemb200_assemble_staged(ctx, sm, phys, beta_re, beta_im, row_begin, row_end, out);
    bemb200_staged_mesh_free(sm);
    return rc;
}

int bemb200_assembly_stats_get(const bemb200_matrix* m, bemb200_assembly_stats* out) {
    if (!m || !out) return set_error(nullptr, BEMB200_EINVAL, "NULL argument");
    *out = m->stats;
    return BEMB200_OK;
}

int bemb200_matrix_from_host(bemb200_ctx* ctx, const double* a_rows, uint64_t n_rows_global, uint64_t n_cols,
                             uint64_t row_begin, uint64_t row_end, bemb200_matrix** out) {
    if (!ctx) return set_error(nullptr, BEMB200_EINVAL, "ctx is NULL");
    if (!a_rows || !out || row_begin > row_end || row_end > n_rows_global || n_cols == 0)
        return set_error(ctx, BEMB200_EINVAL, "bad argument");
    std::lock_guard<std::mutex> lk(ctx->mu);
    BEMB_CUDA(ctx, cudaSetDevice(ctx->device));
    bemb200_matrix* m = nullptr;
    int rc = matrix_alloc(ctx, n_rows_global, n_cols, row_begin, row_end, false, &m);
    if (rc != BEMB200_OK) return rc;
    cudaError_t e = cudaMemcpyAsync(m->A, a_rows, (row_end - row_begin) * n_cols * sizeof(cplx), cudaMemcpyHostToDevice, ctx->stream);
    if (e == cudaSuccess) e = cudaStreamSynchronize(ctx->stream);
    if (e != cudaSuccess) {
        bemb200_matrix_free(m);
        return cuda_fail(ctx, e, "matrix upload");
    }
    *out = m;
    return BEMB200_OK;
}

int bemb200_ctx_set_background(bemb200_ctx* ctx, int blocks_per_sm) {
    if (!ctx || blocks_per_sm < 0 || blocks_per_sm > 8) return set_error(ctx, BEMB200_EINVAL, "blocks_per_sm must be 0..8");
    ctx->background_blocks_per_sm.store(blocks_per_sm);
    return BEMB200_OK;
}

int bemb200_ctx_set_shared_gpu(bemb200_ctx* ctx, int shared) {
    if (!ctx) return set_error(ctx, BEMB200_EINVAL, "NULL context");
    ctx->shared_gpu.store(shared ? 1 : 0);
    return BEMB200_OK;
}

int bemb200_matrix_boost_assembly(bemb200_matrix* m, bemb200_ctx* ctx) {
    if (!m || !ctx) return set_error(ctx, BEMB200_EINVAL, "NULL argument");
    if (ctx->device != m->ctx->device) return set_error(ctx, BEMB200_EINVAL, "contexts must share the device");
    std::lock_guard<std::mutex> lk(ctx->mu);
    std::lock_guard<std::mutex> bl(m->boost_mu);
    if (!m->far_running || m->relaunch.empty() || m->boost_pending) return BEMB200_OK;
    BEMB_CUDA(ctx, cudaSetDevice(ctx->device));
    BEMB_CUDA(ctx, cudaStreamWaitEvent(ctx->stream, m->far_ready_ev, 0));
    for (auto& fn : m->relaunch) BEMB_CUDA(ctx, fn(ctx->stream));
    BEMB_CUDA(ctx, cudaEventRecord(m->boost_ev, ctx->stream));
    m->boost_pending = true;
    return BEMB200_OK;
}

int bemb200_ctx_peer_exchange_active(const bemb200_ctx* ctx, int* active) {
    if (!ctx || !active) return set_error(nullptr, BEMB200_EINVAL, "NULL argument");
    *active = ctx->px.ok ? 1 : 0;
    return BEMB200_OK;
}

int bemb200_matrix_set_context(bemb200_matrix* m, bemb200_ctx* ctx) {
    if (!m || !ctx) return set_error(ctx, BEMB200_EINVAL, "NULL argument");
    if (ctx->device != m->ctx->device || ctx->nranks != m->ctx->nranks || ctx->rank != m->ctx->rank)
        return set_error(ctx, BEMB200_EINVAL, "contexts must share device, rank and nranks");
    std::lock_guard<std::mutex> lk(m->ctx->mu);
    cudaSetDevice(ctx->device);
    cudaStreamSynchronize(m->ctx->stream);
    free_workspace(m);
    m->ctx = ctx;
    return BEMB200_OK;
}

uint64_t bemb200_num_rows(const bemb200_matrix* m) { return m ? m->n_rows : 0; }
uint64_t bemb200_num_cols(const bemb200_matrix* m) { return m ? m->n_cols : 0; }
uint64_t bemb200_local_row_begin(const bemb200_matrix* m) { return m ? m->r0 : 0; }
uint64_t bemb200_local_row_end(const bemb200_matrix* m) { return m ? m->r1 : 0; }
void* bemb200_matrix_device_ptr(const bemb200_matrix* m) { return m ? (void*)m->A : nullptr; }

int bemb200_matrix_download(const bemb200_matrix* m, uint64_t row_begin, uint64_t row_end, double* out) {
    if (!m || !out) return set_error(nullptr, BEMB200_EINVAL, "NULL argument");
    bemb200_ctx* ctx = m->ctx;
    if (row_begin > row_end || row_begin < m->r0 || row_end > m->r1) return set_error(ctx, BEMB200_EINVAL, "rows outside the local slab");
    std::lock_guard<std::mutex> lk(ctx->mu);
    BEMB_CUDA(ctx, cudaSetDevice(ctx->device));
    BEMB_CUDA(ctx, cudaMemcpyAsync(out, m->A + (row_begin - m->r0) * m->n_cols, (row_end - row_begin) * m->n_cols * sizeof(cplx),
                                   cudaMemcpyDeviceToHost, ctx->stream));
    BEMB_CUDA(ctx, cudaStreamSynchronize(ctx->stream));
    return BEMB200_OK;
}

int bemb200_rhs_download(const bemb200_matrix* m, double* out) {
    if (!m || !out) return set_error(nullptr, BEMB200_EINVAL, "NULL argument");
    bemb200_ctx* ctx = m->ctx;
    std::lock_guard<std::mutex> lk(ctx->mu);
    BEMB_CUDA(ctx, cudaSetDevice(ctx->device));
    BEMB_CUDA(ctx, cudaMemcpyAsync(out, m->rhs, (m->r1 - m->r0) * sizeof(cplx), cudaMemcpyDeviceToHost, ctx->stream));
    BEMB_CUDA(ctx, cudaStreamSynchronize(ctx->stream));
    return BEMB200_OK;
}

}
```

### math_audio_b200/csrc/api_internal.h

```cpp
#pragma once
#include <cuda_runtime.h>
#include <atomic>
#include <condition_variable>
#include <memory>
#include <mutex>
#include <string>
#include <vector>

#include "../../include/bemb200.h"
#include "internal.h"

struct PeerExchange {
    bool tried = false, ok = false;
    uint64_t npad = 0;
    unsigned char* local = nullptr;
    unsigned char* base[8] = {nullptr, nullptr, nullptr, nullptr, nullptr, nullptr, nullptr, nullptr};
    unsigned long long epoch = 0;
    int* err_h = nullptr;
};

namespace bemb {
constexpr int MAX_GROUP_RANKS = 8;
struct PeerGroup {
    int nranks = 0;
    int device[MAX_GROUP_RANKS] = {0, 0, 0, 0, 0, 0, 0, 0};
    bool peer_ok = true;
    std::mutex mu;
    std::condition_variable cv;
    unsigned char* posted[MAX_GROUP_RANKS] = {nullptr, nullptr, nullptr, nullptr, nullptr, nullptr, nullptr, nullptr};
    unsigned char* snap[MAX_GROUP_RANKS] = {nullptr, nullptr, nullptr, nullptr, nullptr, nullptr, nullptr, nullptr};
    int arrived = 0;
    unsigned long long generation = 0;
    bool exchange(int rank, unsigned char* mine, unsigned char** all);
};
}

struct FusedLocal {
    uint4* cpart = nullptr;
    uint4* hbuf = nullptr;
    void* result_h = nullptr;
    void* result_d = nullptr;
    int grid = 0;
    uint32_t er = 0;
    bool disabled = false;
    unsigned long long* trace_d = nullptr;
    uint32_t* row_off_d = nullptr;
    uint4* frag = nullptr;
    std::vector<double> speed;
    std::vector<unsigned> smid;
    int calib_runs = 0;
};

struct bemb200_ctx {
    int device = 0;
    int rank = 0, nranks = 1;
    cudaStream_t stream = nullptr;
    bool own_stream = true;
    std::atomic<int> shared_gpu{0};
    std::atomic<int> background_blocks_per_sm{0};
    void* nccl_comm = nullptr;
    PeerExchange px;
    FusedLocal fx;
    std::shared_ptr<bemb::PeerGroup> group;
    int fused_grid = 0;
    std::string err;
    std::mutex mu;
};

struct bemb200_staged_mesh {
    bemb200_ctx* ctx = nullptr;
    bemb::DeviceMesh dm;
    std::vector<void*> allocs;
};

struct GmresWorkspace;

struct bemb200_matrix {
    bemb200_ctx* ctx = nullptr;
    uint64_t n_rows = 0, n_cols = 0;
    uint64_t r0 = 0, r1 = 0;
    bemb::cplx* A = nullptr;
    bemb::cplx* rhs = nullptr;
    uint2* near_list = nullptr;
    unsigned int near_cap = 0;
    unsigned int* near_count = nullptr;
    bemb200_assembly_stats stats{};
    cudaEvent_t ev[4] = {nullptr, nullptr, nullptr, nullptr};
    GmresWorkspace* ws = nullptr;
    unsigned int* work_counters = nullptr;
    std::mutex boost_mu;
    bool far_running = false;
    bool boost_pending = false;
    bemb::FarRelaunch relaunch;
    cudaEvent_t far_ready_ev = nullptr, boost_ev = nullptr;
    uint64_t last_launches = 0, last_matvecs = 0;
    double last_matvec_ms = 0.0;
    double last_solve_ms = 0.0;
};

namespace bemb {
int set_error(bemb200_ctx* ctx, int code, const std::string& msg);
int cuda_fail(bemb200_ctx* ctx, cudaError_t e, const char* what);
void free_workspace(bemb200_matrix* m);
void free_peer_exchange(bemb200_ctx* ctx, bool collective);
}

#define BEMB_CUDA(ctx, call)                                          \
    do {                                                              \
        cudaError_t _e = (call);                                      \
        if (_e != cudaSuccess) return bemb::cuda_fail(ctx, _e, #call); \
    } while (0)
```

### math_audio_b200/csrc/assembly_far.cu

```cuda
#include <atomic>
#include <cmath>
#include <cstdlib>

#include "internal.h"

namespace bemb {

namespace {

struct RuleConst {
    double w[NQ_MAX];
    double a[NQ_MAX];
    double b[NQ_MAX];
    double a2[NQ_MAX];
    double b2[NQ_MAX];
    double ac, bc;
    double ac2, bc2;
    double xi[NQ_MAX];
    double eta[NQ_MAX];
};
__device__ __constant__ RuleConst d_rule_tri;
__device__ __constant__ RuleConst d_rule_quad;
__device__ double2 d_sincos_tab[SINCOS_TAB];

__device__ __forceinline__ uint32_t smem_u32(const void* p) { return (uint32_t)__cvta_generic_to_shared(p); }

template <int NQ, bool BIMAG, int MINB>
__global__ void __launch_bounds__(TILE, MINB)
far_kernel(const double* __restrict__ far_k, const double* __restrict__ far_c, const uint8_t* __restrict__ col_class,
           const double* __restrict__ srcdat, uint32_t n, uint64_t row_begin, uint64_t row_end, uint32_t rows_per_block,
           uint32_t nchunks, uint32_t total_items, uint32_t items_per_block,
           double wavruim, CisConst cis, double k2, double cH, double beta_re, double beta_im, cplx* __restrict__ A, uint64_t lda,
           uint2* __restrict__ near_list, unsigned int near_cap, unsigned int* __restrict__ near_count,
           unsigned int* __restrict__ work_counter) {
    __shared__ __align__(128) double sm_k[NQ * TILE];
    __shared__ uint32_t s_item;
    extern __shared__ __align__(16) double2 sm_tab[];
    __shared__ __align__(8) unsigned long long mbar;

    const uint32_t t = threadIdx.x;
    constexpr uint32_t BYTES = NQ * TILE * sizeof(double);
    constexpr bool QUAD = (NQ == NQ_QUAD);
    const uint8_t want = QUAD ? COL_FLAT_QUAD : COL_FLAT_TRI;
    const RuleConst& rc = QUAD ? d_rule_quad : d_rule_tri;
    const double bk = beta_im * wavruim, bk2 = beta_im * k2, bk3 = 3.0 * bk, b3 = 3.0 * beta_im;

    if (t == 0) {
        asm volatile("mbarrier.init.shared::cta.b64 [%0], 1;" ::"r"(smem_u32(&mbar)));
        asm volatile("fence.mbarrier_init.release.cluster;" ::: "memory");
    }
    for (uint32_t i = t; i < SINCOS_TAB; i += TILE) sm_tab[i] = d_sincos_tab[i];
    __syncthreads();

    const uint32_t item_first = blockIdx.x * items_per_block;
    const uint32_t item_last = (item_first + items_per_block < total_items) ? item_first + items_per_block : total_items;
    uint32_t cur_tile = 0xffffffffu, loads = 0;
    double nyx = 0, nyy = 0, nyz = 0, j4pi = 0, y0x = 0, y0y = 0, y0z = 0, thr = 0, e1x = 0, e1y = 0, e1z = 0, e2x = 0, e2y = 0,
           e2z = 0, kc = 0;
    bool active = false;
    uint32_t col = 0;
    const double* kq = sm_k + t;

    for (uint32_t it = 0;; ++it) {
    uint32_t item;
    if (work_counter) {
        __syncthreads();
        if (t == 0) s_item = atomicAdd(work_counter, 1u);
        __syncthreads();
        item = s_item;
        if (item >= total_items) break;
    } else {
        item = item_first + it;
        if (item >= item_last) break;
    }
    const uint32_t tile = item / nchunks, chunk = item - tile * nchunks;
    if (tile != cur_tile) {
        cur_tile = tile;
        col = tile * TILE + t;
        __syncthreads();
        if (t == 0) {
            const double* gsrc = far_k + (uint64_t)tile * NQ_MAX * TILE;
            asm volatile("mbarrier.arrive.expect_tx.shared::cta.b64 _, [%0], %1;" ::"r"(smem_u32(&mbar)), "r"(BYTES) : "memory");
            asm volatile(
                "cp.async.bulk.shared::cluster.global.mbarrier::complete_tx::bytes [%0], [%1], %2, [%3];" ::"r"(smem_u32(sm_k)),
                "l"(gsrc), "r"(BYTES), "r"(smem_u32(&mbar))
                : "memory");
        }
        const double* fc = far_c + (uint64_t)tile * FAR_NCONST * TILE + t;
        nyx = fc[FC_NX * TILE]; nyy = fc[FC_NY * TILE]; nyz = fc[FC_NZ * TILE];
        j4pi = fc[FC_J4PI * TILE];
        y0x = fc[FC_Y0X * TILE]; y0y = fc[FC_Y0Y * TILE]; y0z = fc[FC_Y0Z * TILE];
        thr = fc[FC_THR * TILE];
        e1x = fc[FC_E1X * TILE]; e1y = fc[FC_E1Y * TILE]; e1z = fc[FC_E1Z * TILE];
        e2x = fc[FC_E2X * TILE]; e2y = fc[FC_E2Y * TILE]; e2z = fc[FC_E2Z * TILE];
        kc = fc[FC_KC * TILE];
        active = (col < n) && (col_class[col] == want);
        {
            const uint32_t parity = loads & 1u;
            uint32_t done = 0;
            while (!done) {
                asm volatile(
                    "{\n .reg .pred p;\n mbarrier.try_wait.parity.shared::cta.b64 p, [%1], %2;\n selp.u32 %0, 1, 0, p;\n}\n"
                    : "=r"(done)
                    : "r"(smem_u32(&mbar)), "r"(parity)
                    : "memory");
            }
            ++loads;
        }
    }

    const uint64_t r0 = row_begin + (uint64_t)chunk * rows_per_block;
    const uint64_t r1 = (r0 + rows_per_block < row_end) ? r0 + rows_per_block : row_end;

    for (uint64_t row = r0; row < r1; ++row) {
        const double* sp = srcdat + 8ull * row;
        const double sx = __ldg(sp + 0), sy = __ldg(sp + 1), sz = __ldg(sp + 2);
        const double nxx = __ldg(sp + 3), nxy = __ldg(sp + 4), nxz = __ldg(sp + 5);
        const double dx = y0x - sx, dy = y0y - sy, dz = y0z - sz;
        const double D = fma(dz, dz, fma(dy, dy, dx * dx));
        const double p1 = fma(dz, e1z, fma(dy, e1y, dx * e1x));
        const double p2 = fma(dz, e2z, fma(dy, e2y, dx * e2x));
        double d2c = D;
        if (QUAD) d2c = fma(rc.ac2, p1, fma(rc.bc2, p2, D + kc));
        const bool is_near = active && (d2c < thr);
        if (__any_sync(0xffffffffu, is_near)) {
            const unsigned mask = __ballot_sync(0xffffffffu, is_near && (uint64_t)col != row);
            if (mask) {
                unsigned base = 0;
                const int leader = __ffs(mask) - 1;
                if ((int)(t & 31) == leader) base = atomicAdd(near_count, __popc(mask));
                base = __shfl_sync(0xffffffffu, base, leader);
                if (is_near && (uint64_t)col != row) {
                    unsigned pos = base + __popc(mask & ((1u << (t & 31)) - 1u));
                    if (pos < near_cap) near_list[pos] = make_uint2((unsigned)row, col);
                }
            }
        }
        const double h = fma(dz, nyz, fma(dy, nyy, dx * nyx));
        const double nn = fma(nxz, nyz, fma(nxy, nyy, nxx * nyx));
        const double M0 = fma(dz, nxz, fma(dy, nxy, dx * nxx));
        const double E1 = fma(e1z, nxz, fma(e1y, nxy, e1x * nxx));
        const double E2 = fma(e2z, nxz, fma(e2y, nxy, e2x * nxx));
        const double nh = -h;
        const double nhc = -cH * h;
        const double hck = (cH * h) * wavruim;
        const double c3 = bk * nn, c2 = beta_im * nn;
        const double bk3nh = bk3 * nh, b3nh = b3 * nh, bk2nh = bk2 * nh;
        double are = 0.0, aim = 0.0;
#pragma unroll
        for (int q = 0; q < NQ; ++q) {
            const double r2 = (q == 0) ? D : fma(rc.a2[q], p1, fma(rc.b2[q], p2, D + kq[q * TILE]));
            const double rho = fast_rsqrt(r2);
            const double r = r2 * rho;
            double sn, cs;
            fast_cis_tab(r, cis, sm_tab, sn, cs);
            const double m = (q == 0) ? M0 : fma(rc.a[q], E1, fma(rc.b[q], E2, M0));
            const double rho2 = rho * rho;
            if (BIMAG) {
                const double X = fma(bk3nh, m * rho2, fma(nhc, rho, c3));
                const double Z = fma(m, fma(b3nh, rho2, -bk2nh), c2);
                const double Y = fma(rho, Z, hck);
                const double G = rc.w[q] * rho2;
                are = fma(G, fma(cs, X, -(sn * Y)), are);
                aim = fma(G, fma(cs, Y, sn * X), aim);
            } else {
                const double g = rho * rc.w[q];
                const double zgr = g * cs, zgi = g * sn;
                const double rq = (nh * m) * rho2;
                const double t3 = fma(3.0, rq, nn);
                const double A1 = nhc * rho2;
                const double A2 = hck * rho;
                const double P = fma(rho2, t3, -(k2 * rq));
                const double Q = (wavruim * rho) * t3;
                const double fre = fma(beta_re, P, fma(beta_im, Q, A1));
                const double fim = fma(beta_im, P, fma(-beta_re, Q, A2));
                are = fma(zgr, fre, fma(-zgi, fim, are));
                aim = fma(zgr, fim, fma(zgi, fre, aim));
            }
        }
        if (active) {
            double2 v = make_double2(are * j4pi, aim * j4pi);
            __stcs(reinterpret_cast<double2*>(A + (row - row_begin) * lda + col), v);
        }
    }
    }
}


template <int NQ>
__global__ void __launch_bounds__(256)
rhs_far_kernel(const double* __restrict__ far_k, const double* __restrict__ far_c, const uint32_t* __restrict__ cols, uint32_t ncols,
               const double* __restrict__ srcdat, const cplx* __restrict__ bc_val, const uint8_t* __restrict__ bc_len,
               uint64_t row_begin, uint64_t row_end, double wavruim, double gamtau, cplx beta0, cplx* __restrict__ rhs) {
    constexpr bool QUAD = (NQ == NQ_QUAD);
    const RuleConst& rc = QUAD ? d_rule_quad : d_rule_tri;
    const int lane = threadIdx.x & 31;
    const uint64_t row = row_begin + (((uint64_t)blockIdx.x * blockDim.x + threadIdx.x) >> 5);
    if (row >= row_end) return;
    const double* sp = srcdat + 8ull * row;
    const double sx = sp[0], sy = sp[1], sz = sp[2], nxx = sp[3], nxy = sp[4], nxz = sp[5];
    double accr = 0.0, acci = 0.0;
    for (uint32_t ci = lane; ci < ncols; ci += 32) {
        const uint32_t col = cols[ci];
        if ((uint64_t)col == row) continue;
        const uint32_t tile = col / TILE, t = col % TILE;
        const double* fc = far_c + (uint64_t)tile * FAR_NCONST * TILE + t;
        const double* fk = far_k + (uint64_t)tile * NQ_MAX * TILE + t;
        const double dx = fc[FC_Y0X * TILE] - sx, dy = fc[FC_Y0Y * TILE] - sy, dz = fc[FC_Y0Z * TILE] - sz;
        const double e1x = fc[FC_E1X * TILE], e1y = fc[FC_E1Y * TILE], e1z = fc[FC_E1Z * TILE];
        const double e2x = fc[FC_E2X * TILE], e2y = fc[FC_E2Y * TILE], e2z = fc[FC_E2Z * TILE];
        const double D = fma(dz, dz, fma(dy, dy, dx * dx));
        const double p1 = fma(dz, e1z, fma(dy, e1y, dx * e1x));
        const double p2 = fma(dz, e2z, fma(dy, e2y, dx * e2x));
        double d2c = D;
        if (QUAD) d2c = fma(rc.ac2, p1, fma(rc.bc2, p2, D + fc[FC_KC * TILE]));
        if (d2c < fc[FC_THR * TILE]) continue;
        const double M0 = fma(dz, nxz, fma(dy, nxy, dx * nxx));
        const double E1 = fma(e1z, nxz, fma(e1y, nxy, e1x * nxx));
        const double E2 = fma(e2z, nxz, fma(e2y, nxy, e2x * nxx));
        const int bl = bc_len[col];
        cplx bc[4];
#pragma unroll
        for (int i = 0; i < 4; ++i) bc[i] = i < bl ? bc_val[4ull * col + i] : C(0, 0);
        double pr = 0.0, pi = 0.0;
#pragma unroll
        for (int q = 0; q < NQ; ++q) {
            const double r2 = (q == 0) ? D : fma(rc.a2[q], p1, fma(rc.b2[q], p2, D + fk[q * TILE]));
            const double rho = fast_rsqrt(r2);
            const double r = r2 * rho;
            double sn, cs;
            fast_sincos(wavruim * r, sn, cs);
            const double m = (q == 0) ? M0 : fma(rc.a[q], E1, fma(rc.b[q], E2, M0));
            double N[4];
            if (QUAD) {
                const double s1 = 0.25 * (rc.xi[q] + 1.0), s2 = 0.25 * (rc.xi[q] - 1.0), t1 = rc.eta[q] + 1.0, t2 = rc.eta[q] - 1.0;
                N[0] = s1 * t1; N[1] = -s2 * t1; N[2] = s2 * t2; N[3] = -s1 * t2;
            } else {
                N[0] = 1.0 - rc.xi[q] - rc.eta[q]; N[1] = rc.xi[q]; N[2] = rc.eta[q]; N[3] = 0.0;
            }
            double zr = 0.0, zi = 0.0;
#pragma unroll
            for (int i = 0; i < 4; ++i) { zr = fma(bc[i].re, N[i], zr); zi = fma(bc[i].im, N[i], zi); }
            const double g = rc.w[q] * rho;
            const double gr = g * cs, gi = g * sn;
            const double hr = m * rho * rho, hi = -wavruim * m * rho;
            const double tr = gr * hr - gi * hi, ti = gr * hi + gi * hr;
            const double fr = gr * gamtau + (tr * beta0.re - ti * beta0.im), fi = gi * gamtau + (tr * beta0.im + ti * beta0.re);
            pr += fr * zr - fi * zi;
            pi += fr * zi + fi * zr;
        }
        const double j4pi = fc[FC_J4PI * TILE];
        accr = fma(pr, j4pi, accr);
        acci = fma(pi, j4pi, acci);
    }
#pragma unroll
    for (int mm = 16; mm >= 1; mm >>= 1) {
        accr += __shfl_xor_sync(0xffffffffu, accr, mm);
        acci += __shfl_xor_sync(0xffffffffu, acci, mm);
    }
    if (lane == 0) {
        atomicAdd(&rhs[row - row_begin].re, accr);
        atomicAdd(&rhs[row - row_begin].im, acci);
    }
}

bool g_tables_uploaded[64] = {false};

cudaError_t upload_tables() {
    int dev = 0;
    cudaError_t e = cudaGetDevice(&dev);
    if (e != cudaSuccess) return e;
    if (dev < 64 && g_tables_uploaded[dev]) return cudaSuccess;
    RuleConst tri = {}, quad = {};
    for (int q = 0; q < NQ_TRI; ++q) {
        tri.w[q] = hosttab::BEMQ_TR13[q][2] * 0.5;
        tri.a[q] = hosttab::BEMQ_TR13[q][0] - hosttab::BEMQ_TR13[0][0];
        tri.b[q] = hosttab::BEMQ_TR13[q][1] - hosttab::BEMQ_TR13[0][1];
        tri.xi[q] = hosttab::BEMQ_TR13[q][0];
        tri.eta[q] = hosttab::BEMQ_TR13[q][1];
    }
    tri.ac = 0.0; tri.bc = 0.0;
    for (int i = 0; i < 4; ++i)
        for (int j = 0; j < 4; ++j) {
            const int q = i * 4 + j;
            quad.w[q] = hosttab::BEMQ_GL4_W[i] * hosttab::BEMQ_GL4_W[j];
            quad.a[q] = hosttab::BEMQ_GL4_X[i] - hosttab::BEMQ_GL4_X[0];
            quad.b[q] = hosttab::BEMQ_GL4_X[j] - hosttab::BEMQ_GL4_X[0];
            quad.xi[q] = hosttab::BEMQ_GL4_X[i];
            quad.eta[q] = hosttab::BEMQ_GL4_X[j];
        }
    quad.ac = -hosttab::BEMQ_GL4_X[0]; quad.bc = -hosttab::BEMQ_GL4_X[0];
    for (RuleConst* r : {&tri, &quad}) {
        for (int q = 0; q < NQ_MAX; ++q) { r->a2[q] = 2.0 * r->a[q]; r->b2[q] = 2.0 * r->b[q]; }
        r->ac2 = 2.0 * r->ac; r->bc2 = 2.0 * r->bc;
    }
    {
        double2 tab[SINCOS_TAB];
        for (int i = 0; i < SINCOS_TAB; ++i) {
            const long double ang = (long double)i * (3.14159265358979323846264338327950288L / (long double)SINCOS_STEPS_PER_PI);
            tab[i] = make_double2((double)cosl(ang), (double)sinl(ang));
        }
        tab[0] = make_double2(1.0, 0.0); tab[SINCOS_TAB / 4] = make_double2(0.0, 1.0);
        tab[SINCOS_TAB / 2] = make_double2(-1.0, 0.0); tab[3 * SINCOS_TAB / 4] = make_double2(0.0, -1.0);
        e = cudaMemcpyToSymbol(d_sincos_tab, tab, sizeof tab);
        if (e != cudaSuccess) return e;
    }
    e = cudaMemcpyToSymbol(d_rule_tri, &tri, sizeof tri);
    if (e != cudaSuccess) return e;
    e = cudaMemcpyToSymbol(d_rule_quad, &quad, sizeof quad);
    if (e != cudaSuccess) return e;
    if (dev < 64) g_tables_uploaded[dev] = true;
    return cudaSuccess;
}

int env_int(const char* name, int dflt) {
    const char* v = std::getenv(name);
    return v ? std::atoi(v) : dflt;
}

template <int NQ, bool BIMAG, int MINB>
cudaError_t launch_far_v(const DeviceMesh& m, const Phys& ph, uint64_t row_begin, uint64_t row_end, cplx* A, uint64_t lda,
                         uint2* near_list, unsigned int near_cap, unsigned int* near_count, int background_blocks_per_sm,
                         unsigned int* work_counter, FarRelaunch* relaunch, cudaStream_t s) {
    const uint64_t nrows = row_end - row_begin;
    uint32_t rpb = 128;
    while (rpb > 8 && (uint64_t)m.ntiles * ((nrows + rpb - 1) / rpb) < 148ull * MINB * 4ull) rpb >>= 1;
    const uint32_t nchunks = (uint32_t)((nrows + rpb - 1) / rpb);
    const uint32_t total = m.ntiles * nchunks;
    uint32_t grid = total, ipb = 1;
    unsigned int* counter = nullptr;
    if (background_blocks_per_sm > 0 && total > 148u * (uint32_t)background_blocks_per_sm) {
        grid = 148u * (uint32_t)background_blocks_per_sm;
        ipb = (total + grid - 1) / grid;
        grid = (total + ipb - 1) / ipb;
        counter = work_counter;
    }
    const double cH = ph.sign * ph.gamma * ph.tau;
    const double *far_k = m.far_k, *far_c = m.far_c, *src = m.src;
    const uint8_t* col_class = m.col_class;
    const uint32_t n = m.n;
    const double wavruim = ph.wavruim, k2 = ph.k2, bre = ph.beta.re, bim = ph.beta.im;
    const CisConst cis = make_cis_const(ph.wavruim);
    constexpr size_t TAB_BYTES = SINCOS_TAB * sizeof(double2);
    {
        static std::atomic<unsigned char> attr_done[64];
        int dev = 0;
        cudaGetDevice(&dev);
        if (dev < 0 || dev >= 64) dev = 63;
        if (!attr_done[dev].load()) {
            cudaError_t ae = cudaFuncSetAttribute(far_kernel<NQ, BIMAG, MINB>, cudaFuncAttributeMaxDynamicSharedMemorySize, (int)TAB_BYTES);
            if (ae != cudaSuccess) return ae;
            attr_done[dev].store(1);
        }
    }
    auto launch = [=](cudaStream_t st, unsigned int g, unsigned int* ctr) -> cudaError_t {
        far_kernel<NQ, BIMAG, MINB><<<g, TILE, TAB_BYTES, st>>>(far_k, far_c, col_class, src, n, row_begin, row_end, rpb, nchunks, total, ipb,
                                                       wavruim, cis, k2, cH, bre, bim, A, lda, near_list, near_cap, near_count, ctr);
        return cudaGetLastError();
    };
    if (counter && relaunch) {
        const unsigned int hg = total < 148u * 4u ? total : 148u * 4u;
        relaunch->push_back([=](cudaStream_t st) { return launch(st, hg, counter); });
    }
    return launch(s, grid, counter);
}

template <int NQ>
cudaError_t launch_far_t(const DeviceMesh& m, const Phys& ph, uint64_t row_begin, uint64_t row_end, cplx* A, uint64_t lda,
                         uint2* near_list, unsigned int near_cap, unsigned int* near_count, int bg, unsigned int* work_counter,
                         FarRelaunch* relaunch, cudaStream_t s) {
    const bool bimag = (ph.beta.re == 0.0);
    static const int minb = env_int("BEMB200_FAR_MINB", 4);
#define FAR_DISPATCH(B, M) \
    return launch_far_v<NQ, B, M>(m, ph, row_begin, row_end, A, lda, near_list, near_cap, near_count, bg, work_counter, relaunch, s)
    if (bimag) {
        if (minb == 2) FAR_DISPATCH(true, 2);
        if (minb == 3) FAR_DISPATCH(true, 3);
        if (minb == 5) FAR_DISPATCH(true, 5);
        if (minb == 6) FAR_DISPATCH(true, 6);
        FAR_DISPATCH(true, 4);
    }
    FAR_DISPATCH(false, 4);
#undef FAR_DISPATCH
}

}

cudaError_t launch_rhs_far(const DeviceMesh& m, const Phys& ph, uint64_t row_begin, uint64_t row_end, cplx* rhs, cudaStream_t s) {
    if (row_end <= row_begin || (m.n_rhs_tri == 0 && m.n_rhs_quad == 0)) return cudaSuccess;
    cudaError_t e = upload_tables();
    if (e != cudaSuccess) return e;
    const uint64_t nrows = row_end - row_begin;
    const unsigned blocks = (unsigned)((nrows * 32 + 255) / 256);
    const double gamtau = ph.gamma * ph.tau;
    if (m.n_rhs_tri)
        rhs_far_kernel<NQ_TRI><<<blocks, 256, 0, s>>>(m.far_k, m.far_c, m.rhs_cols_tri, m.n_rhs_tri, m.src, m.bc_val, m.bc_len, row_begin,
                                                     row_end, ph.wavruim, gamtau, ph.beta_unscaled, rhs);
    if (m.n_rhs_quad)
        rhs_far_kernel<NQ_QUAD><<<blocks, 256, 0, s>>>(m.far_k, m.far_c, m.rhs_cols_quad, m.n_rhs_quad, m.src, m.bc_val, m.bc_len, row_begin,
                                                      row_end, ph.wavruim, gamtau, ph.beta_unscaled, rhs);
    return cudaGetLastError();
}

int far_kernel_launch_count(const DeviceMesh& m) { return (m.n_flat_tri ? 1 : 0) + (m.n_flat_quad ? 1 : 0); }

cudaError_t launch_far(const DeviceMesh& m, const Phys& ph, uint64_t row_begin, uint64_t row_end, cplx* A, uint64_t lda,
                       uint2* near_list, unsigned int near_cap, unsigned int* near_count, int background_blocks_per_sm,
                       unsigned int* work_counters, FarRelaunch* relaunch, cudaStream_t s) {
    if (row_end <= row_begin) return cudaSuccess;
    cudaError_t e = upload_tables();
    if (e != cudaSuccess) return e;
    if (m.n_flat_tri) {
        e = launch_far_t<NQ_TRI>(m, ph, row_begin, row_end, A, lda, near_list, near_cap, near_count, background_blocks_per_sm,
                                 work_counters ? work_counters + 0 : nullptr, relaunch, s);
        if (e != cudaSuccess) return e;
    }
    if (m.n_flat_quad) {
        e = launch_far_t<NQ_QUAD>(m, ph, row_begin, row_end, A, lda, near_list, near_cap, near_count, background_blocks_per_sm,
                                  work_counters ? work_counters + 1 : nullptr, relaunch, s);
        if (e != cudaSuccess) return e;
    }
    return cudaSuccess;
}

}
```

### math_audio_b200/csrc/internal.h

```cpp
#pragma once
#include <cuda_runtime.h>
#include <stdint.h>
#include <functional>
#include <mutex>
#include <string>
#include <vector>

#include "common.cuh"

namespace bemb {

struct DeviceMesh {
    uint32_t n = 0;
    uint32_t ntiles = 0;
    double* coords = nullptr;
    uint8_t* etype = nullptr;
    double* area = nullptr;
    double* src = nullptr;
    int32_t* bc_type = nullptr;
    uint8_t* bc_len = nullptr;
    cplx* bc_val = nullptr;
    uint8_t* nonzero_bc = nullptr;
    double* esize = nullptr;
    double* far_k = nullptr;
    double* far_c = nullptr;
    uint8_t* col_class = nullptr;
    uint32_t* special_cols = nullptr;
    uint32_t n_special = 0;
    uint32_t n_flat_tri = 0, n_flat_quad = 0;
    uint32_t* rhs_cols_tri = nullptr;
    uint32_t* rhs_cols_quad = nullptr;
    uint32_t n_rhs_tri = 0, n_rhs_quad = 0;
    double avg_radius_first100 = 0.0;
};

struct Phys {
    double k;
    double wavruim;
    double k2;
    double tau, gamma;
    double sign;
    cplx beta;
    cplx beta_unscaled;
};

struct AssemblyStats {
    unsigned long long near_pairs = 0;
    unsigned long long far_pairs = 0;
    unsigned long long special_pairs = 0;
    unsigned int near_overflow = 0;
};

cudaError_t launch_prep(const DeviceMesh& m, cudaStream_t s);
typedef std::vector<std::function<cudaError_t(cudaStream_t)>> FarRelaunch;
cudaError_t launch_far(const DeviceMesh& m, const Phys& ph, uint64_t row_begin, uint64_t row_end, cplx* A, uint64_t lda,
                       uint2* near_list, unsigned int near_cap, unsigned int* near_count, int background_blocks_per_sm,
                       unsigned int* work_counters, FarRelaunch* relaunch, cudaStream_t s);
cudaError_t launch_rhs_far(const DeviceMesh& m, const Phys& ph, uint64_t row_begin, uint64_t row_end, cplx* rhs, cudaStream_t s);
cudaError_t launch_near_list(const DeviceMesh& m, const Phys& ph, uint64_t row_begin, cplx* A, uint64_t lda, cplx* rhs,
                             const uint2* near_list, unsigned int count, cudaStream_t s);
cudaError_t launch_special(const DeviceMesh& m, const Phys& ph, uint64_t row_begin, uint64_t row_end, cplx* A,
                           uint64_t lda, cplx* rhs, cudaStream_t s);
cudaError_t launch_self(const DeviceMesh& m, const Phys& ph, uint64_t row_begin, uint64_t row_end, cplx* A, uint64_t lda,
                        cplx* rhs, cudaStream_t s);
int far_kernel_launch_count(const DeviceMesh& m);

}
```

### math_audio_b200/csrc/sweep.cu

```cuda
#include <condition_variable>
#include <cstring>
#include <deque>
#include <memory>
#include <thread>

#include "api_internal.h"

using namespace bemb;

struct SweepJob {
    bemb200_physics phys;
    double beta_re, beta_im;
    std::vector<double> rhs_extra;
    uint32_t max_iterations, restart;
    double tolerance;
    int slot = 0;
    int rc = BEMB200_OK;
    std::string err;
    bool assembled = false;
};

struct bemb200_sweep {
    bemb200_ctx* ctx_solve = nullptr;
    bemb200_ctx* ctx_asm = nullptr;
    bemb200_staged_mesh* staged = nullptr;
    bemb200_matrix* buf[2] = {nullptr, nullptr};
    bool buf_handed[2] = {false, false};
    uint64_t n = 0, r0 = 0, r1 = 0;
    bool overlap = true;
    int background = 1;
    std::thread worker;
    std::mutex mu;
    std::condition_variable cv;
    std::deque<std::shared_ptr<SweepJob>> queue;
    size_t next_to_assemble = 0;
    bool slot_busy[2] = {false, false};
    bool solving = false;
    bool stop = false;
    uint64_t submitted = 0, boosts = 0;
    std::string err;
    bool precond = false;
    uint32_t pc_subdomains = 0;
    std::vector<uint64_t> pc_ptr, pc_idx;
    double pc_setup_ms = 0.0;
};

static void sweep_worker(bemb200_sweep* sw) {
    cudaSetDevice(sw->ctx_asm->device);
    for (;;) {
        std::shared_ptr<SweepJob> job;
        bool foreground;
        {
            std::unique_lock<std::mutex> lk(sw->mu);
            sw->cv.wait(lk, [&] {
                if (sw->stop) return true;
                if (sw->next_to_assemble >= sw->queue.size()) return false;
                return !sw->slot_busy[sw->queue[sw->next_to_assemble]->slot];
            });
            if (sw->stop) return;
            job = sw->queue[sw->next_to_assemble];
            sw->next_to_assemble += 1;
            sw->slot_busy[job->slot] = true;
            foreground = job == sw->queue.front();
        }
        bemb200_ctx_set_background(sw->ctx_asm, (sw->overlap && !foreground) ? sw->background : 0);
        int rc = bemb200_assemble_staged(sw->ctx_asm, sw->staged, &job->phys, job->beta_re, job->beta_im, sw->r0, sw->r1, &sw->buf[job->slot]);
        if (rc == BEMB200_OK && sw->overlap && !sw->buf_handed[job->slot]) {
            rc = bemb200_matrix_set_context(sw->buf[job->slot], sw->ctx_solve);
            sw->buf_handed[job->slot] = rc == BEMB200_OK;
        }
        {
            std::lock_guard<std::mutex> lk(sw->mu);
            job->rc = rc;
            if (rc != BEMB200_OK) job->err = bemb200_last_error(sw->ctx_asm);
            job->assembled = true;
        }
        sw->cv.notify_all();
    }
}

extern "C" {

int bemb200_sweep_create(int device, int rank, int nranks, const uint8_t* nccl_id, const bemb200_mesh* mesh, int overlap,
                         int background_blocks_per_sm, bemb200_sweep** out) {
    if (!out || !mesh) return set_error(nullptr, BEMB200_EINVAL, "NULL argument");
    *out = nullptr;
    std::unique_ptr<bemb200_sweep> sw(new bemb200_sweep());
    sw->overlap = overlap != 0;
    sw->background = background_blocks_per_sm > 0 ? background_blocks_per_sm : 1;
    int rc = bemb200_ctx_create_ex(device, rank, nranks, nccl_id, nullptr, &sw->ctx_solve);
    if (rc != BEMB200_OK) return rc;
    if (sw->overlap) {
        rc = bemb200_ctx_create_ex(device, rank, nranks, nullptr, nullptr, &sw->ctx_asm);
        if (rc != BEMB200_OK) { bemb200_ctx_destroy(sw->ctx_solve); return rc; }
    } else {
        sw->ctx_asm = sw->ctx_solve;
    }
    rc = bemb200_mesh_stage(sw->ctx_asm, mesh, &sw->staged);
    if (rc != BEMB200_OK) {
        const std::string msg = bemb200_last_error(sw->ctx_asm);
        if (sw->overlap) bemb200_ctx_destroy(sw->ctx_asm);
        bemb200_ctx_destroy(sw->ctx_solve);
        return set_error(nullptr, rc, msg);
    }
    sw->n = bemb200_staged_num_dofs(sw->staged);
    bemb200_partition(sw->n, nranks, rank, &sw->r0, &sw->r1);
    bemb200_sweep* raw = sw.release();
    raw->worker = std::thread(sweep_worker, raw);
    *out = raw;
    return BEMB200_OK;
}

uint64_t bemb200_sweep_num_dofs(const bemb200_sweep* sw) { return sw ? sw->n : 0; }

int bemb200_sweep_submit(bemb200_sweep* sw, const bemb200_physics* phys, double beta_re, double beta_im, const double* rhs_extra,
                         uint32_t max_iterations, uint32_t restart, double tolerance) {
    if (!sw || !phys) return set_error(nullptr, BEMB200_EINVAL, "NULL argument");
    if (restart == 0) return set_error(sw->ctx_solve, BEMB200_EINVAL, "restart must be >= 1");
    auto job = std::make_shared<SweepJob>();
    job->phys = *phys;
    job->beta_re = beta_re;
    job->beta_im = beta_im;
    if (rhs_extra) job->rhs_extra.assign(rhs_extra, rhs_extra + 2 * sw->n);
    job->max_iterations = max_iterations;
    job->restart = restart;
    job->tolerance = tolerance;
    {
        std::lock_guard<std::mutex> lk(sw->mu);
        job->slot = (int)(sw->submitted & 1u);
        sw->submitted += 1;
        sw->queue.push_back(job);
    }
    sw->cv.notify_all();
    return BEMB200_OK;
}

int bemb200_sweep_next(bemb200_sweep* sw, double* x_out, bemb200_gmres_info* info, bemb200_assembly_stats* stats, double* rhs_out) {
    if (!sw || !x_out || !info) return set_error(nullptr, BEMB200_EINVAL, "NULL argument");
    std::shared_ptr<SweepJob> job;
    {
        std::unique_lock<std::mutex> lk(sw->mu);
        if (sw->queue.empty()) return set_error(sw->ctx_solve, BEMB200_EINVAL, "bemb200_sweep_next: nothing submitted");
        job = sw->queue.front();
        sw->cv.wait(lk, [&] { return job->assembled; });
        if (job->rc != BEMB200_OK) {
            sw->queue.pop_front();
            sw->next_to_assemble -= 1;
            sw->slot_busy[job->slot] = false;
            sw->cv.notify_all();
            return set_error(sw->ctx_solve, job->rc, job->err);
        }
        sw->solving = true;
        bemb200_ctx_set_shared_gpu(sw->ctx_solve, (sw->overlap && sw->queue.size() > 1) ? 1 : 0);
    }
    bemb200_matrix* m = sw->buf[job->slot];
    int rc = BEMB200_OK;
    if (stats) rc = bemb200_assembly_stats_get(m, stats);
    std::vector<double> b(2 * sw->n);
    if (rc == BEMB200_OK) rc = bemb200_rhs_download_full(m, b.data());
    if (rc == BEMB200_OK) {
        if (!job->rhs_extra.empty())
            for (size_t i = 0; i < b.size(); ++i) b[i] += job->rhs_extra[i];
        if (rhs_out) std::memcpy(rhs_out, b.data(), b.size() * sizeof(double));
        bool use_pc;
        uint32_t nsub;
        std::vector<uint64_t> pptr, pidx;
        {
            std::lock_guard<std::mutex> lk(sw->mu);
            use_pc = sw->precond; nsub = sw->pc_subdomains; pptr = sw->pc_ptr; pidx = sw->pc_idx;
        }
        if (!use_pc) {
            rc = bemb200_gmres(m, b.data(), nullptr, job->max_iterations, job->restart, job->tolerance, x_out, info);
        } else {
            bemb200_precond* pc = nullptr;
            rc = bemb200_schwarz_create(m, nsub, pptr.empty() ? nullptr : pptr.data(), pptr.empty() ? nullptr : pidx.data(), &pc);
            if (rc == BEMB200_OK) {
                bemb200_precond_stats st{};
                if (bemb200_precond_stats_get(pc, &st) == BEMB200_OK) sw->pc_setup_ms = st.factor_ms;
                rc = bemb200_gmres_schwarz(m, pc, b.data(), nullptr, job->max_iterations, job->restart, job->tolerance, x_out, info);
            }
            bemb200_precond_free(pc);
        }
    }
    bool boost = false;
    {
        std::lock_guard<std::mutex> lk(sw->mu);
        sw->solving = false;
        bemb200_ctx_set_shared_gpu(sw->ctx_solve, 0);
        sw->queue.pop_front();
        sw->next_to_assemble -= 1;
        sw->slot_busy[job->slot] = false;
        boost = sw->overlap && !sw->queue.empty() && !sw->queue.front()->assembled && sw->buf[sw->queue.front()->slot] != nullptr;
    }
    sw->cv.notify_all();
    if (boost) {
        std::shared_ptr<SweepJob> nxt;
        {
            std::lock_guard<std::mutex> lk(sw->mu);
            if (!sw->queue.empty()) nxt = sw->queue.front();
        }
        if (nxt && sw->buf[nxt->slot] && bemb200_matrix_boost_assembly(sw->buf[nxt->slot], sw->ctx_solve) == BEMB200_OK) sw->boosts += 1;
    }
    return rc;
}

uint64_t bemb200_sweep_boosts(const bemb200_sweep* sw) { return sw ? sw->boosts : 0; }

int bemb200_sweep_set_block_jacobi(bemb200_sweep* sw, uint32_t num_subdomains, const uint64_t* sub_ptr, const uint64_t* sub_idx) {
    if (!sw) return set_error(nullptr, BEMB200_EINVAL, "NULL argument");
    if ((sub_ptr == nullptr) != (sub_idx == nullptr)) return set_error(sw->ctx_solve, BEMB200_EINVAL, "sub_ptr and sub_idx go together");
    std::lock_guard<std::mutex> lk(sw->mu);
    sw->precond = num_subdomains > 0;
    sw->pc_subdomains = num_subdomains;
    sw->pc_ptr.clear(); sw->pc_idx.clear();
    if (sw->precond && sub_ptr) {
        sw->pc_ptr.assign(sub_ptr, sub_ptr + num_subdomains + 1);
        sw->pc_idx.assign(sub_idx, sub_idx + sub_ptr[num_subdomains]);
    }
    return BEMB200_OK;
}

void bemb200_sweep_destroy(bemb200_sweep* sw) {
    if (!sw) return;
    {
        std::lock_guard<std::mutex> lk(sw->mu);
        sw->stop = true;
    }
    sw->cv.notify_all();
    if (sw->worker.joinable()) sw->worker.join();
    for (int i = 0; i < 2; ++i)
        if (sw->buf[i]) bemb200_matrix_free(sw->buf[i]);
    if (sw->staged) bemb200_staged_mesh_free(sw->staged);
    if (sw->overlap && sw->ctx_asm) bemb200_ctx_destroy(sw->ctx_asm);
    if (sw->ctx_solve) bemb200_ctx_destroy(sw->ctx_solve);
    delete sw;
}

}

struct bemb200_multi {
    int n = 0;
    std::vector<int> devices;
    std::vector<bemb200_ctx*> ctx;
    std::shared_ptr<bemb::PeerGroup> group;
    std::string err;
};
struct bemb200_multi_matrix {
    bemb200_multi* mg = nullptr;
    std::vector<bemb200_matrix*> m;
    uint64_t n = 0;
};

template <class F>
static int on_all_ranks(bemb200_multi* mg, F fn) {
    std::vector<int> rc(mg->n, BEMB200_OK);
    std::vector<std::thread> th;
    for (int p = 0; p < mg->n; ++p) th.emplace_back([&, p] { rc[p] = fn(p); });
    for (auto& t : th) t.join();
    for (int p = 0; p < mg->n; ++p)
        if (rc[p] != BEMB200_OK) {
            mg->err = bemb200_last_error(mg->ctx[p]);
            return set_error(nullptr, rc[p], mg->err);
        }
    return BEMB200_OK;
}

extern "C" {

int bemb200_multi_create(const int* devices, int n, bemb200_multi** out) {
    if (!devices || !out || n < 1 || n > MAX_GROUP_RANKS) return set_error(nullptr, BEMB200_EINVAL, "bemb200_multi_create: 1..8 devices");
    *out = nullptr;
    std::unique_ptr<bemb200_multi> mg(new bemb200_multi());
    mg->n = n;
    mg->devices.assign(devices, devices + n);
    mg->group = std::make_shared<bemb::PeerGroup>();
    mg->group->nranks = n;
    for (int p = 0; p < n; ++p) mg->group->device[p] = devices[p];
    for (int p = 0; p < n; ++p) {
        bemb200_ctx* c = nullptr;
        int rc = bemb200_ctx_create_ex(devices[p], p, n, nullptr, nullptr, &c);
        if (rc != BEMB200_OK) {
            for (bemb200_ctx* q : mg->ctx) bemb200_ctx_destroy(q);
            return rc;
        }
        c->group = mg->group;
        int same = 0;
        for (int q = 0; q < n; ++q) same += devices[q] == devices[p] ? 1 : 0;
        if (same > 1) {
            int sms = 0;
            cudaDeviceGetAttribute(&sms, cudaDevAttrMultiProcessorCount, devices[p]);
            c->fused_grid = sms / same;
        }
        mg->ctx.push_back(c);
    }
    for (int p = 0; p < n; ++p)
        for (int q = 0; q < n; ++q)
            if (devices[p] != devices[q]) {
                cudaSetDevice(devices[p]);
                cudaError_t e = cudaDeviceEnablePeerAccess(devices[q], 0);
                if (e != cudaSuccess && e != cudaErrorPeerAccessAlreadyEnabled) mg->group->peer_ok = false;
                cudaGetLastError();
            }
    *out = mg.release();
    return BEMB200_OK;
}

void bemb200_multi_destroy(bemb200_multi* mg) {
    if (!mg) return;
    for (bemb200_ctx* c : mg->ctx) bemb200_ctx_destroy(c);
    delete mg;
}

int bemb200_multi_num_ranks(const bemb200_multi* mg) { return mg ? mg->n : 0; }
const char* bemb200_multi_last_error(const bemb200_multi* mg) { return mg ? mg->err.c_str() : ""; }

int bemb200_multi_assemble(bemb200_multi* mg, const bemb200_mesh* mesh, const bemb200_physics* phys, double beta_re, double beta_im,
                           bemb200_multi_matrix** out) {
    if (!mg || !mesh || !phys || !out) return set_error(nullptr, BEMB200_EINVAL, "NULL argument");
    *out = nullptr;
    std::unique_ptr<bemb200_multi_matrix> mm(new bemb200_multi_matrix());
    mm->mg = mg;
    mm->m.assign(mg->n, nullptr);
    uint64_t ndof = 0;
    for (uint64_t e = 0; e < mesh->n_elem; ++e) ndof += mesh->is_eval[e] ? 0 : 1;
    mm->n = ndof;
    int rc = on_all_ranks(mg, [&](int p) {
        uint64_t b = 0, e = 0;
        bemb200_partition(ndof, mg->n, p, &b, &e);
        return bemb200_assemble(mg->ctx[p], mesh, phys, beta_re, beta_im, b, e, &mm->m[p]);
    });
    if (rc != BEMB200_OK) {
        for (bemb200_matrix* m : mm->m)
            if (m) bemb200_matrix_free(m);
        return rc;
    }
    *out = mm.release();
    return BEMB200_OK;
}

void bemb200_multi_matrix_free(bemb200_multi_matrix* mm) {
    if (!mm) return;
    for (bemb200_matrix* m : mm->m)
        if (m) bemb200_matrix_free(m);
    delete mm;
}

uint64_t bemb200_multi_num_rows(const bemb200_multi_matrix* mm) { return mm ? mm->n : 0; }

int bemb200_multi_rhs_download(const bemb200_multi_matrix* mm, double* out) {
    if (!mm || !out) return set_error(nullptr, BEMB200_EINVAL, "NULL argument");
    for (int p = 0; p < mm->mg->n; ++p) {
        const uint64_t b = bemb200_local_row_begin(mm->m[p]);
        int rc = bemb200_rhs_download(mm->m[p], out + 2 * b);
        if (rc != BEMB200_OK) return rc;
    }
    return BEMB200_OK;
}

int bemb200_multi_matrix_download(const bemb200_multi_matrix* mm, uint64_t row_begin, uint64_t row_end, double* out) {
    if (!mm || !out || row_begin > row_end || row_end > mm->n) return set_error(nullptr, BEMB200_EINVAL, "bad argument");
    for (int p = 0; p < mm->mg->n; ++p) {
        const uint64_t b = bemb200_local_row_begin(mm->m[p]), e = bemb200_local_row_end(mm->m[p]);
        const uint64_t lo = row_begin > b ? row_begin : b, hi = row_end < e ? row_end : e;
        if (lo >= hi) continue;
        int rc = bemb200_matrix_download(mm->m[p], lo, hi, out + 2 * (lo - row_begin) * mm->n);
        if (rc != BEMB200_OK) return rc;
    }
    return BEMB200_OK;
}

int bemb200_multi_gmres(const bemb200_multi_matrix* mm, const double* b, const double* x0, uint32_t max_iterations, uint32_t restart,
                        double tolerance, double* x_out, bemb200_gmres_info* info) {
    if (!mm || !b || !x_out || !info) return set_error(nullptr, BEMB200_EINVAL, "NULL argument");
    bemb200_multi* mg = mm->mg;
    std::vector<bemb200_gmres_info> infos(mg->n);
    std::vector<std::vector<double>> xs(mg->n);
    int rc = on_all_ranks(mg, [&](int p) {
        xs[p].resize(p == 0 ? 0 : 2 * mm->n);
        return bemb200_gmres(mm->m[p], b, x0, max_iterations, restart, tolerance, p == 0 ? x_out : xs[p].data(), &infos[p]);
    });
    if (rc != BEMB200_OK) return rc;
    *info = infos[0];
    return BEMB200_OK;
}

}
```

### math_audio_b200/sweep.py

```python
from __future__ import annotations

import os
import threading
import time
from typing import Callable, List, Optional, Sequence, Tuple

import numpy as np

from . import bem
from .mesh import Mesh
from .types import PhysicsParams


class Sweep:

    def __init__(self, mesh: Mesh, device: int = 0, rank: int = 0, nranks: int = 1, nccl_id: Optional[bytes] = None,
                 overlap: bool = True, background_blocks_per_sm: int = 2):
        import ctypes as C

        from . import _capi

        self._capi, self._C = _capi, C
        self._lib = _capi.lib()
        self._h = C.c_void_p()
        cm = _capi.cmesh(mesh)
        idbuf = (C.c_uint8 * 128).from_buffer_copy(nccl_id) if nccl_id else None
        _capi.check(self._lib.bemb200_sweep_create(device, rank, nranks, idbuf, C.byref(cm), 1 if overlap else 0,
                                                   background_blocks_per_sm, C.byref(self._h)), None)
        self.n = int(self._lib.bemb200_sweep_num_dofs(self._h))
        self.mesh_nbytes = _capi.mesh_nbytes(mesh)

    def submit(self, physics: PhysicsParams, beta: complex, rhs_extra: Optional[np.ndarray], config: "bem.GmresConfig") -> None:
        ph = bem._cphys(physics)
        beta = complex(beta)
        extra = None
        if rhs_extra is not None:
            extra = np.ascontiguousarray(rhs_extra, dtype=np.complex128)
            if extra.shape != (self.n,):
                raise ValueError("rhs_extra has the wrong length")
        self._capi.check(self._lib.bemb200_sweep_submit(self._h, self._C.byref(ph), beta.real, beta.imag,
                                                        self._capi.ptr(extra) if extra is not None else None,
                                                        config.max_iterations, config.restart, config.tolerance), None)

    def next(self):
        x = np.empty(self.n, dtype=np.complex128)
        b = np.empty(self.n, dtype=np.complex128)
        info = self._capi.CGmresInfo()
        st = self._capi.CAssemblyStats()
        self._capi.check(self._lib.bemb200_sweep_next(self._h, self._capi.ptr(x), self._C.byref(info), self._C.byref(st),
                                                      self._capi.ptr(b)), None)
        sol = bem.GmresSolution(x=x, iterations=int(info.iterations), restarts=int(info.restarts), residual=float(info.residual),
                                converged=bool(info.converged))
        return sol, {k: getattr(st, k) for k, _ in st._fields_}, b

    def solve_all(self, cases, config: "bem.GmresConfig") -> list:
        out = []
        for c in cases[:2]:
            self.submit(c[0], c[1], c[2], config)
        for i in range(len(cases)):
            out.append(self.next())
            if i + 2 < len(cases):
                c = cases[i + 2]
                self.submit(c[0], c[1], c[2], config)
        return out

    def set_block_jacobi(self, num_subdomains: int = 0, subdomains=None) -> None:
        if subdomains is None:
            self._capi.check(self._lib.bemb200_sweep_set_block_jacobi(self._h, int(num_subdomains), None, None), None)
            return
        ptr = np.zeros(len(subdomains) + 1, dtype=np.uint64)
        ptr[1:] = np.cumsum([len(p) for p in subdomains])
        idx = np.ascontiguousarray(np.concatenate([np.asarray(p, dtype=np.uint64) for p in subdomains]))
        self._capi.check(self._lib.bemb200_sweep_set_block_jacobi(self._h, len(subdomains), self._capi.ptr(ptr), self._capi.ptr(idx)), None)

    @property
    def boosts(self) -> int:
        return int(self._lib.bemb200_sweep_boosts(self._h))

    def close(self):
        if self._h:
            self._lib.bemb200_sweep_destroy(self._h)
            self._h = self._C.c_void_p()

    def __del__(self):
        try:
            self.close()
        except Exception:
            pass


class SweepDriver:

    def __init__(self, mesh: Mesh, device: int = 0, rank: int = 0, nranks: int = 1, nccl_id: Optional[bytes] = None,
                 solve_stream: int = 0, assembly_stream: int = 0, overlap: bool = True, background_blocks_per_sm: int = 2):
        self.ctx_solve = bem.Context(device, rank, nranks, nccl_id, cuda_stream=solve_stream)
        self.ctx_asm = bem.Context(device, rank, nranks, None, cuda_stream=assembly_stream) if overlap else self.ctx_solve
        self.overlap = overlap
        self.background_blocks_per_sm = background_blocks_per_sm if overlap else 0
        self.mesh = mesh
        self.staged = bem.StagedMesh(mesh, self.ctx_asm)
        self.n = self.staged.num_dofs
        self.rows = self.ctx_solve.partition(self.n)
        self.buffers: List[Optional[bem.TbemSystem]] = [None, None]
        self.asm_stats: List[dict] = []
        self.sol_stats: List[dict] = []
        self.boosts = 0
        self.boost = os.environ.get("BEMB200_SWEEP_BOOST", "1") != "0"
        self.trace: Optional[list] = [] if os.environ.get("BEMB200_SWEEP_TRACE") else None
        self._t0 = 0.0

    def _mark(self, label: str, i: int) -> None:
        if self.trace is not None:
            self.trace.append((label, i, time.perf_counter() - self._t0))

    def _assemble(self, slot: int, physics: PhysicsParams, beta: complex, mesh_for_stage: Optional[Mesh], err: list, case: int = -1):
        try:
            self._mark("asm_begin", case)
            staged = self.staged if mesh_for_stage is None else bem.StagedMesh(mesh_for_stage, self.ctx_asm)
            self._mark("asm_staged", case)
            first = self.buffers[slot] is None
            self.buffers[slot] = bem.build_tbem_system_with_beta(staged, physics, beta, ctx=self.ctx_asm, rows=self.rows,
                                                                reuse=self.buffers[slot], fetch_rhs=False)
            if first and self.overlap:
                self.buffers[slot].matrix.set_context(self.ctx_solve)
            self._mark("asm_end", case)
        except Exception as e:
            err.append(e)

    def run(self, cases: Sequence[Tuple[PhysicsParams, complex]], config: bem.GmresConfig,
            solve: Callable[[int, bem.TbemSystem, bem.DenseOperator], object], restage_host_mesh: bool = False) -> list:
        out = []
        err: list = []
        mesh_arg = self.mesh if restage_host_mesh else None
        if not cases:
            return out
        self._t0 = time.perf_counter()
        self.ctx_asm.set_background(0)
        self._assemble(0, cases[0][0], cases[0][1], mesh_arg, err, 0)
        if err:
            raise err[0]
        self.ctx_asm.set_background(self.background_blocks_per_sm)
        self.ctx_solve.set_shared_gpu(self.overlap)
        try:
            for i in range(len(cases)):
                t = None
                if i + 1 < len(cases):
                    if self.overlap:
                        t = threading.Thread(target=self._assemble, args=((i + 1) % 2, cases[i + 1][0], cases[i + 1][1], mesh_arg, err, i + 1))
                        t.start()
                elif self.overlap:
                    self.ctx_solve.set_shared_gpu(False)
                system = self.buffers[i % 2]
                self.asm_stats.append(system.matrix.assembly_stats())
                op = bem.DenseOperator(system)
                self._mark("solve_begin", i)
                out.append(solve(i, system, op))
                self._mark("solve_end", i)
                self.sol_stats.append(system.matrix.solver_stats())
                if t is not None:
                    nxt = self.buffers[(i + 1) % 2]
                    if self.boost and nxt is not None and t.is_alive():
                        nxt.matrix.boost_assembly(self.ctx_solve)
                        self.boosts += 1
                    t.join()
                    self._mark("joined", i)
                elif i + 1 < len(cases):
                    self._assemble((i + 1) % 2, cases[i + 1][0], cases[i + 1][1], mesh_arg, err, i + 1)
                if err:
                    raise err[0]
        finally:
            self.ctx_solve.set_shared_gpu(False)
        return out
```

### rust/bem-b200-sys/src/lib.rs

```rust
#![allow(non_camel_case_types)]
use std::os::raw::{c_char, c_double, c_int, c_void};

#[repr(C)] pub struct bemb200_ctx { _p: [u8; 0] }
#[repr(C)] pub struct bemb200_staged_mesh { _p: [u8; 0] }
#[repr(C)] pub struct bemb200_matrix { _p: [u8; 0] }
#[repr(C)] pub struct bemb200_sweep { _p: [u8; 0] }
#[repr(C)] pub struct bemb200_precond { _p: [u8; 0] }
#[repr(C)] #[derive(Clone, Copy, Default)]
pub struct bemb200_precond_stats { pub num_subdomains: u32, pub local_subdomains: u32, pub min_size: u32, pub max_size: u32,
                                   pub avg_size: f64, pub inverse_bytes: u64, pub factor_ms: f64, pub disjoint: i32 }
#[repr(C)] pub struct bemb200_multi { _p: [u8; 0] }
#[repr(C)] pub struct bemb200_multi_matrix { _p: [u8; 0] }
#[repr(C)] #[derive(Clone, Copy, Default)]
pub struct bemb200_assembly_stats { pub near_pairs: u64, pub special_pairs: u64, pub far_kernel_launches: u64,
                                    pub total_launches: u64, pub far_ms: f64, pub total_ms: f64 }

#[repr(C)]
pub struct bemb200_mesh {
    pub n_nodes: u64, pub n_elem: u64,
    pub nodes: *const f64, pub conn: *const u32, pub etype: *const u8,
    pub center: *const f64, pub normal: *const f64, pub area: *const f64,
    pub bc_type: *const i32, pub bc_len: *const u8, pub bc_val: *const f64,
    pub dof: *const u32, pub is_eval: *const u8,
}
#[repr(C)] #[derive(Clone, Copy)]
pub struct bemb200_physics { pub wave_number: f64, pub harmonic_factor: f64, pub tau: f64, pub gamma: f64 }
pub type bemb200_precond_fn = Option<unsafe extern "C" fn(user: *mut c_void, r: *const f64, z: *mut f64, n: u64) -> c_int>;
#[repr(C)] #[derive(Clone, Copy, Default)]
pub struct bemb200_gmres_info { pub iterations: u64, pub restarts: u64, pub residual: f64, pub converged: i32 }

extern "C" {
    pub fn bemb200_ctx_create(device: c_int, out: *mut *mut bemb200_ctx) -> c_int;
    pub fn bemb200_ctx_create_ex(device: c_int, rank: c_int, nranks: c_int, nccl_id: *const u8,
                                 cuda_stream: *mut c_void, out: *mut *mut bemb200_ctx) -> c_int;
    pub fn bemb200_nccl_unique_id(out: *mut u8) -> c_int;
    pub fn bemb200_ctx_destroy(ctx: *mut bemb200_ctx);
    pub fn bemb200_ctx_set_background(ctx: *mut bemb200_ctx, blocks_per_sm: c_int) -> c_int;
    pub fn bemb200_ctx_set_shared_gpu(ctx: *mut bemb200_ctx, shared: c_int) -> c_int;
    pub fn bemb200_ctx_peer_exchange_active(ctx: *const bemb200_ctx, active: *mut c_int) -> c_int;
    pub fn bemb200_last_error(ctx: *const bemb200_ctx) -> *const c_char;
    pub fn bemb200_partition(n: u64, nranks: c_int, rank: c_int, row_begin: *mut u64, row_end: *mut u64);
    pub fn bemb200_mesh_stage(ctx: *mut bemb200_ctx, mesh: *const bemb200_mesh, out: *mut *mut bemb200_staged_mesh) -> c_int;
    pub fn bemb200_staged_mesh_free(sm: *mut bemb200_staged_mesh);
    pub fn bemb200_assemble_staged(ctx: *mut bemb200_ctx, sm: *const bemb200_staged_mesh, phys: *const bemb200_physics,
                                   beta_re: c_double, beta_im: c_double, row_begin: u64, row_end: u64,
                                   inout: *mut *mut bemb200_matrix) -> c_int;
    pub fn bemb200_assemble(ctx: *mut bemb200_ctx, mesh: *const bemb200_mesh, phys: *const bemb200_physics,
                            beta_re: c_double, beta_im: c_double, row_begin: u64, row_end: u64,
                            out: *mut *mut bemb200_matrix) -> c_int;
    pub fn bemb200_matrix_from_host(ctx: *mut bemb200_ctx, a_rows: *const f64, n_rows_global: u64, n_cols: u64,
                                    row_begin: u64, row_end: u64, out: *mut *mut bemb200_matrix) -> c_int;
    pub fn bemb200_matrix_free(m: *mut bemb200_matrix);
    pub fn bemb200_num_rows(m: *const bemb200_matrix) -> u64;
    pub fn bemb200_num_cols(m: *const bemb200_matrix) -> u64;
    pub fn bemb200_matrix_download(m: *const bemb200_matrix, row_begin: u64, row_end: u64, out: *mut f64) -> c_int;
    pub fn bemb200_rhs_download_full(m: *const bemb200_matrix, out: *mut f64) -> c_int;
    pub fn bemb200_row_sum_correction(m: *mut bemb200_matrix, avg: *mut f64) -> c_int;
    pub fn bemb200_apply(m: *const bemb200_matrix, x: *const f64, y: *mut f64) -> c_int;
    pub fn bemb200_apply_transpose(m: *const bemb200_matrix, x: *const f64, y: *mut f64) -> c_int;
    pub fn bemb200_bicgstab(m: *const bemb200_matrix, b: *const f64, max_iterations: u32, tolerance: f64, x_out: *mut f64,
                            info: *mut bemb200_gmres_info) -> c_int;
    pub fn bemb200_cgs(m: *const bemb200_matrix, b: *const f64, max_iterations: u32, tolerance: f64, x_out: *mut f64,
                       info: *mut bemb200_gmres_info) -> c_int;
    pub fn bemb200_lu_solve(m: *const bemb200_matrix, b: *const f64, x_out: *mut f64, overwrite_matrix: c_int,
                            factor_ms: *mut f64) -> c_int;
    pub fn bemb200_compute_rcs(sm: *const bemb200_staged_mesh, phys: *const bemb200_physics, n_dirs: u32, dirs: *const f64,
                               surface_pressure: *const f64, rcs_out: *mut f64) -> c_int;
    pub fn bemb200_gmres_preconditioned(m: *const bemb200_matrix, inv_diag: *const f64, b: *const f64, x0: *const f64,
                                        max_iterations: u32, restart: u32, tolerance: f64, x_out: *mut f64,
                                        info: *mut bemb200_gmres_info) -> c_int;
    pub fn bemb200_matrix_diagonal(m: *const bemb200_matrix, out: *mut f64) -> c_int;
    pub fn bemb200_schwarz_create(m: *const bemb200_matrix, num_subdomains: u32, sub_ptr: *const u64, sub_idx: *const u64,
                                  out: *mut *mut bemb200_precond) -> c_int;
    pub fn bemb200_precond_free(p: *mut bemb200_precond);
    pub fn bemb200_precond_stats_get(p: *const bemb200_precond, out: *mut bemb200_precond_stats) -> c_int;
    pub fn bemb200_precond_apply(p: *const bemb200_precond, r: *const f64, z: *mut f64) -> c_int;
    pub fn bemb200_gmres_schwarz(m: *const bemb200_matrix, precond: *const bemb200_precond, b: *const f64, x0: *const f64,
                                 max_iterations: u32, restart: u32, tolerance: f64, x_out: *mut f64,
                                 info: *mut bemb200_gmres_info) -> c_int;
    pub fn bemb200_gmres_callback(m: *const bemb200_matrix, apply: bemb200_precond_fn, user: *mut c_void, b: *const f64, x0: *const f64,
                                  max_iterations: u32, restart: u32, tolerance: f64, x_out: *mut f64, info: *mut bemb200_gmres_info,
                                  precond_calls: *mut u64) -> c_int;
    pub fn bemb200_gmres_batched(m: *const bemb200_matrix, b_all: *const f64, nrhs: u32, max_iterations: u32, restart: u32,
                                 tolerance: f64, x_all: *mut f64, infos: *mut bemb200_gmres_info, block_matvec_ms: *mut f64,
                                 block_matvecs: *mut u64) -> c_int;
    pub fn bemb200_gmres_batched_schwarz(m: *const bemb200_matrix, precond: *const bemb200_precond, b_all: *const f64, nrhs: u32,
                                         max_iterations: u32, restart: u32, tolerance: f64, x_all: *mut f64,
                                         infos: *mut bemb200_gmres_info, block_matvec_ms: *mut f64, block_matvecs: *mut u64) -> c_int;
    pub fn bemb200_incident_rhs(sm: *const bemb200_staged_mesh, phys: *const bemb200_physics, beta_re: f64, beta_im: f64,
                                n_sources: u32, kinds: *const i32, vecs: *const f64, amps: *const f64, rhs_host: *mut f64,
                                rhs_dev: *mut f64) -> c_int;
    pub fn bemb200_scattered_field(sm: *const bemb200_staged_mesh, phys: *const bemb200_physics, n_eval: u64, eval_pts: *const f64,
                                   surface_pressure: *const f64, surface_velocity: *const f64, out: *mut f64) -> c_int;
    pub fn bemb200_gmres(m: *const bemb200_matrix, b: *const f64, x0: *const f64, max_iterations: u32, restart: u32,
                         tolerance: f64, x_out: *mut f64, info: *mut bemb200_gmres_info) -> c_int;
    pub fn bemb200_sweep_create(device: c_int, rank: c_int, nranks: c_int, nccl_id: *const u8, mesh: *const bemb200_mesh,
                                overlap: c_int, background_blocks_per_sm: c_int, out: *mut *mut bemb200_sweep) -> c_int;
    pub fn bemb200_sweep_num_dofs(sw: *const bemb200_sweep) -> u64;
    pub fn bemb200_sweep_submit(sw: *mut bemb200_sweep, phys: *const bemb200_physics, beta_re: c_double, beta_im: c_double,
                                rhs_extra: *const f64, max_iterations: u32, restart: u32, tolerance: f64) -> c_int;
    pub fn bemb200_sweep_next(sw: *mut bemb200_sweep, x_out: *mut f64, info: *mut bemb200_gmres_info,
                              stats: *mut bemb200_assembly_stats, rhs_out: *mut f64) -> c_int;
    pub fn bemb200_sweep_boosts(sw: *const bemb200_sweep) -> u64;
    pub fn bemb200_sweep_set_block_jacobi(sw: *mut bemb200_sweep, num_subdomains: u32, sub_ptr: *const u64, sub_idx: *const u64) -> c_int;
    pub fn bemb200_sweep_destroy(sw: *mut bemb200_sweep);
    pub fn bemb200_multi_create(devices: *const c_int, n: c_int, out: *mut *mut bemb200_multi) -> c_int;
    pub fn bemb200_multi_destroy(mg: *mut bemb200_multi);
    pub fn bemb200_multi_last_error(mg: *const bemb200_multi) -> *const c_char;
    pub fn bemb200_multi_assemble(mg: *mut bemb200_multi, mesh: *const bemb200_mesh, phys: *const bemb200_physics,
                                  beta_re: c_double, beta_im: c_double, out: *mut *mut bemb200_multi_matrix) -> c_int;
    pub fn bemb200_multi_matrix_free(mm: *mut bemb200_multi_matrix);
    pub fn bemb200_multi_num_rows(mm: *const bemb200_multi_matrix) -> u64;
    pub fn bemb200_multi_rhs_download(mm: *const bemb200_multi_matrix, out: *mut f64) -> c_int;
    pub fn bemb200_multi_gmres(mm: *const bemb200_multi_matrix, b: *const f64, x0: *const f64, max_iterations: u32, restart: u32,
                               tolerance: f64, x_out: *mut f64, info: *mut bemb200_gmres_info) -> c_int;
}
```

Before: 0.1089.

## Run background assembly in a green-context SM partition during sweep overlap

When background assembly is enabled, the code creates a CUDA green context holding about a quarter of the SMs and runs the far-field assembly on a stream inside it. Event joins keep ordering with the main stream. Because the assembly is now confined to its own SMs, the solver context no longer switches to shared-GPU mode, which is meant to let GMRES on the main stream avoid contention with the overlapped assembly of the next frequency. The risks are a smaller SM budget for assembly, extra event synchronisation, and a dependency on driver green-context support, with a fallback to the old path if that support is missing.

Result: no change. 0.1083, median of 6 (-0.6%).

```diff
diff --git a/include/bemb200.h b/include/bemb200.h
--- a/include/bemb200.h
+++ b/include/bemb200.h
@@ -58,6 +58,8 @@
     uint64_t total_launches;
     double far_ms;
     double total_ms;
+    int32_t partition_sms;
+    int32_t partition_refused;
 } bemb200_assembly_stats;
 
 int bemb200_device_count(void);
@@ -67,6 +69,7 @@
 int bemb200_ctx_create_ex(int device, int rank, int nranks, const uint8_t* nccl_id, void* cuda_stream, bemb200_ctx** out);
 void bemb200_ctx_destroy(bemb200_ctx* ctx);
 int bemb200_ctx_set_background(bemb200_ctx* ctx, int blocks_per_sm);
+int bemb200_ctx_sm_partition(bemb200_ctx* ctx, int* sms);
 int bemb200_ctx_set_shared_gpu(bemb200_ctx* ctx, int shared);
 int bemb200_matrix_boost_assembly(bemb200_matrix* m, bemb200_ctx* ctx);
 int bemb200_ctx_peer_exchange_active(const bemb200_ctx* ctx, int* active);
diff --git a/include/bemb200.hpp b/include/bemb200.hpp
--- a/include/bemb200.hpp
+++ b/include/bemb200.hpp
@@ -91,6 +91,11 @@
     bemb200_ctx* handle() const { return h_; }
     void set_background(int blocks_per_sm) { check(bemb200_ctx_set_background(h_, blocks_per_sm), h_); }
     void set_shared_gpu(bool shared) { check(bemb200_ctx_set_shared_gpu(h_, shared ? 1 : 0), h_); }
+    int sm_partition() {
+        int sms = 0;
+        check(bemb200_ctx_sm_partition(h_, &sms), h_);
+        return sms;
+    }
     bool peer_exchange_active() const {
         int a = 0;
         check(bemb200_ctx_peer_exchange_active(h_, &a), h_);
diff --git a/math_audio_b200/_capi.py b/math_audio_b200/_capi.py
--- a/math_audio_b200/_capi.py
+++ b/math_audio_b200/_capi.py
@@ -38,7 +38,8 @@
 
 class CAssemblyStats(C.Structure):
     _fields_ = [("near_pairs", C.c_uint64), ("special_pairs", C.c_uint64), ("far_kernel_launches", C.c_uint64),
-                ("total_launches", C.c_uint64), ("far_ms", C.c_double), ("total_ms", C.c_double)]
+                ("total_launches", C.c_uint64), ("far_ms", C.c_double), ("total_ms", C.c_double),
+                ("partition_sms", C.c_int32), ("partition_refused", C.c_int32)]
 
 
 class CPrecondStats(C.Structure):
@@ -65,6 +66,7 @@
     "bemb200_matrix_set_context": (C.c_int, [_VP, _VP]),
     "bemb200_ctx_set_background": (C.c_int, [_VP, C.c_int]),
     "bemb200_ctx_set_shared_gpu": (C.c_int, [_VP, C.c_int]),
+    "bemb200_ctx_sm_partition": (C.c_int, [_VP, C.POINTER(C.c_int)]),
     "bemb200_matrix_boost_assembly": (C.c_int, [_VP, _VP]),
     "bemb200_ctx_peer_exchange_active": (C.c_int, [_VP, C.POINTER(C.c_int)]),
     "bemb200_last_error": (C.c_char_p, [_VP]),
diff --git a/math_audio_b200/bem.py b/math_audio_b200/bem.py
--- a/math_audio_b200/bem.py
+++ b/math_audio_b200/bem.py
@@ -48,6 +48,11 @@
 
     def set_background(self, blocks_per_sm: int) -> None:
         _capi.check(self._lib.bemb200_ctx_set_background(self._h, blocks_per_sm), self._h)
+
+    def sm_partition(self) -> int:
+        k = C.c_int(0)
+        _capi.check(self._lib.bemb200_ctx_sm_partition(self._h, C.byref(k)), self._h)
+        return int(k.value)
 
     def peer_exchange_active(self) -> bool:
         a = C.c_int(0)
diff --git a/math_audio_b200/csrc/api.cu b/math_audio_b200/csrc/api.cu
--- a/math_audio_b200/csrc/api.cu
+++ b/math_audio_b200/csrc/api.cu
@@ -1,7 +1,11 @@
 #include <cmath>
 #include <cstdio>
+#include <cstdlib>
 #include <cstring>
 #include <dlfcn.h>
+
+#include <cuda.h>
+#include <cudaTypedefs.h>
 
 #include "api_internal.h"
 
@@ -77,6 +81,125 @@
 }
 }
 
+namespace {
+struct GreenApi {
+    PFN_cuDeviceGet_v2000 DeviceGet = nullptr;
+    PFN_cuDeviceGetDevResource_v12040 GetDevResource = nullptr;
+    PFN_cuDevSmResourceSplitByCount_v12040 SplitByCount = nullptr;
+    PFN_cuDevResourceGenerateDesc_v12040 GenerateDesc = nullptr;
+    PFN_cuGreenCtxCreate_v12040 CtxCreate = nullptr;
+    PFN_cuGreenCtxDestroy_v12040 CtxDestroy = nullptr;
+    PFN_cuGreenCtxStreamCreate_v12050 StreamCreate = nullptr;
+    PFN_cuStreamDestroy_v4000 StreamDestroy = nullptr;
+    bool ok = false;
+};
+
+template <class F>
+bool driver_entry(const char* name, unsigned int version, F* fn) {
+    void* p = nullptr;
+    cudaDriverEntryPointQueryResult q = cudaDriverEntryPointSymbolNotFound;
+    if (cudaGetDriverEntryPointByVersion(name, &p, version, cudaEnableDefault, &q) != cudaSuccess || q != cudaDriverEntryPointSuccess || !p) {
+        cudaGetLastError();
+        return false;
+    }
+    *fn = reinterpret_cast<F>(p);
+    return true;
+}
+
+const GreenApi& green_api() {
+    static const GreenApi api = []() {
+        GreenApi a;
+        a.ok = driver_entry("cuDeviceGet", 2000, &a.DeviceGet) && driver_entry("cuDeviceGetDevResource", 12040, &a.GetDevResource) &&
+               driver_entry("cuDevSmResourceSplitByCount", 12040, &a.SplitByCount) &&
+               driver_entry("cuDevResourceGenerateDesc", 12040, &a.GenerateDesc) && driver_entry("cuGreenCtxCreate", 12040, &a.CtxCreate) &&
+               driver_entry("cuGreenCtxDestroy", 12040, &a.CtxDestroy) && driver_entry("cuGreenCtxStreamCreate", 12050, &a.StreamCreate) &&
+               driver_entry("cuStreamDestroy", 4000, &a.StreamDestroy);
+        return a;
+    }();
+    return api;
+}
+
+constexpr int SMS_PER_PARTITION_NUM = 27, SMS_PER_PARTITION_DEN = 100;
+int partition_request(int device) {
+    if (const char* v = std::getenv("BEMB200_SWEEP_SM_PARTITION")) return std::atoi(v);
+    int sms = 0;
+    if (cudaDeviceGetAttribute(&sms, cudaDevAttrMultiProcessorCount, device) != cudaSuccess) {
+        cudaGetLastError();
+        return 0;
+    }
+    const int k = (sms * SMS_PER_PARTITION_NUM / SMS_PER_PARTITION_DEN + 4) / 8 * 8;
+    return k < 8 ? 8 : k;
+}
+
+void partition_destroy(bemb200_ctx* ctx) {
+    const GreenApi& g = green_api();
+    if (ctx->part_stream) {
+        cudaStreamSynchronize(ctx->part_stream);
+        g.StreamDestroy((CUstream)ctx->part_stream);
+    }
+    if (ctx->part_green) g.CtxDestroy((CUgreenCtx)ctx->part_green);
+    for (cudaEvent_t& e : ctx->part_join)
+        if (e) cudaEventDestroy(e);
+    ctx->part_stream = nullptr;
+    ctx->part_green = nullptr;
+    ctx->part_join[0] = ctx->part_join[1] = nullptr;
+    ctx->part_sms = 0;
+    cudaGetLastError();
+}
+
+bool partition_create(bemb200_ctx* ctx, int want) {
+    const GreenApi& g = green_api();
+    int sms = 0;
+    if (!g.ok || cudaDeviceGetAttribute(&sms, cudaDevAttrMultiProcessorCount, ctx->device) != cudaSuccess || want >= sms) return false;
+    CUdevice dev = 0;
+    CUdevResource all{}, part{}, rest{};
+    unsigned int groups = 1;
+    CUdevResourceDesc desc = nullptr;
+    CUgreenCtx green = nullptr;
+    CUstream st = nullptr;
+    if (g.DeviceGet(&dev, ctx->device) != CUDA_SUCCESS || g.GetDevResource(dev, &all, CU_DEV_RESOURCE_TYPE_SM) != CUDA_SUCCESS ||
+        g.SplitByCount(&part, &groups, &all, &rest, 0, (unsigned int)want) != CUDA_SUCCESS || groups < 1 ||
+        part.sm.smCount == 0 || part.sm.smCount >= (unsigned int)sms || g.GenerateDesc(&desc, &part, 1) != CUDA_SUCCESS ||
+        g.CtxCreate(&green, desc, dev, CU_GREEN_CTX_DEFAULT_STREAM) != CUDA_SUCCESS)
+        return false;
+    ctx->part_green = green;
+    if (g.StreamCreate(&st, green, CU_STREAM_NON_BLOCKING, 0) != CUDA_SUCCESS) {
+        partition_destroy(ctx);
+        return false;
+    }
+    ctx->part_stream = (cudaStream_t)st;
+    ctx->part_sms = (int)part.sm.smCount;
+    bool ok = cudaEventCreateWithFlags(&ctx->part_join[0], cudaEventDisableTiming) == cudaSuccess &&
+              cudaEventCreateWithFlags(&ctx->part_join[1], cudaEventDisableTiming) == cudaSuccess &&
+              cudaEventRecord(ctx->part_join[0], ctx->stream) == cudaSuccess &&
+              cudaStreamWaitEvent(ctx->part_stream, ctx->part_join[0], 0) == cudaSuccess &&
+              cudaEventRecord(ctx->part_join[1], ctx->part_stream) == cudaSuccess &&
+              cudaStreamWaitEvent(ctx->stream, ctx->part_join[1], 0) == cudaSuccess && cudaStreamSynchronize(ctx->stream) == cudaSuccess;
+    if (!ok) partition_destroy(ctx);
+    return ok;
+}
+
+__global__ void smid_kernel(unsigned int* ids) {
+    unsigned int id;
+    asm volatile("mov.u32 %0, %%smid;" : "=r"(id));
+    const long long t0 = clock64();
+    while (clock64() - t0 < 20000) {}
+    if (threadIdx.x == 0) ids[blockIdx.x] = id;
+}
+}
+
+namespace bemb {
+int ctx_ensure_partition(bemb200_ctx* ctx) {
+    std::lock_guard<std::mutex> lk(ctx->part_mu);
+    if (!ctx->part_tried) {
+        ctx->part_tried = true;
+        const int want = partition_request(ctx->device);
+        if (want > 0 && !partition_create(ctx, want)) ctx->part_refused = true;
+    }
+    return ctx->part_sms;
+}
+}
+
 template <class T>
 static int dev_alloc_copy(bemb200_staged_mesh* sm, T** dst, const std::vector<T>& src) {
     size_t bytes = src.size() * sizeof(T);
@@ -184,6 +307,7 @@
     if (!ctx) return;
     cudaSetDevice(ctx->device);
     free_peer_exchange(ctx, false);
+    partition_destroy(ctx);
     if (ctx->nccl_comm && ncclshim::CommDestroy) ncclshim::CommDestroy(ctx->nccl_comm);
     if (ctx->stream && ctx->own_stream) cudaStreamDestroy(ctx->stream);
     delete ctx;
@@ -422,7 +546,9 @@
     ph.beta = C(beta_re, beta_im);
     ph.beta_unscaled = phys->tau > 0.0 ? C(0.0, phys->harmonic_factor / phys->wave_number) : C(0.0, 0.0);
     const uint64_t nloc = row_end - row_begin;
-    cudaStream_t s = ctx->stream;
+    const bool background = ctx->background_blocks_per_sm.load() > 0;
+    const int part = background ? ctx_ensure_partition(ctx) : 0;
+    cudaStream_t s = part ? ctx->part_stream : ctx->stream;
     int rc = BEMB200_OK;
     unsigned int count = 0;
     auto fail = [&](int code) {
@@ -434,6 +560,10 @@
         cudaError_t _e = (call);                                       \
         if (_e != cudaSuccess) return fail(cuda_fail(ctx, _e, #call)); \
     } while (0)
+    if (part) {
+        ASM_CUDA(cudaEventRecord(ctx->part_join[0], ctx->stream));
+        ASM_CUDA(cudaStreamWaitEvent(s, ctx->part_join[0], 0));
+    }
     ASM_CUDA(cudaMemsetAsync(m->rhs, 0, (nloc + 1) * sizeof(cplx), s));
     if (dm.n_special) ASM_CUDA(cudaMemsetAsync(m->A, 0, nloc * dm.n * sizeof(cplx), s));
     ASM_CUDA(cudaEventRecord(m->ev[0], s));
@@ -450,8 +580,9 @@
             std::lock_guard<std::mutex> bl(m->boost_mu);
             m->relaunch.clear();
             m->boost_pending = false;
-            cudaError_t fe = launch_far(dm, ph, row_begin, row_end, m->A, dm.n, m->near_list, m->near_cap, m->near_count, bg,
-                                        boostable ? m->work_counters : nullptr, boostable ? &m->relaunch : nullptr, s);
+            const int bg_sms = bg > 0 ? (part ? part : 148) : 0;
+            cudaError_t fe = launch_far(dm, ph, row_begin, row_end, m->A, dm.n, m->near_list, m->near_cap, m->near_count, bg_sms,
+                                        part ? 0 : bg, boostable ? m->work_counters : nullptr, boostable ? &m->relaunch : nullptr, s);
             if (fe != cudaSuccess) return fail(cuda_fail(ctx, fe, "launch_far"));
             m->far_running = boostable;
         }
@@ -471,6 +602,7 @@
                 ASM_CUDA(cudaEventSynchronize(m->boost_ev));
                 ASM_CUDA(cudaMemcpyAsync(&count, m->near_count, sizeof(unsigned int), cudaMemcpyDeviceToHost, s));
                 ASM_CUDA(cudaStreamSynchronize(s));
+                s = ctx->stream;
             }
         }
         if (count <= m->near_cap) break;
@@ -488,6 +620,10 @@
     ASM_CUDA(launch_special(dm, ph, row_begin, row_end, m->A, dm.n, m->rhs, s));
     ASM_CUDA(launch_self(dm, ph, row_begin, row_end, m->A, dm.n, m->rhs, s));
     ASM_CUDA(cudaEventRecord(m->ev[3], s));
+    if (s != ctx->stream) {
+        ASM_CUDA(cudaEventRecord(ctx->part_join[1], s));
+        ASM_CUDA(cudaStreamWaitEvent(ctx->stream, ctx->part_join[1], 0));
+    }
     ASM_CUDA(cudaStreamSynchronize(s));
 #undef ASM_CUDA
     float far_ms = 0.f, tot_ms = 0.f;
@@ -500,6 +636,8 @@
                               (dm.n_rhs_tri ? 1 : 0) + (dm.n_rhs_quad ? 1 : 0);
     m->stats.far_ms = far_ms;
     m->stats.total_ms = tot_ms;
+    m->stats.partition_sms = part;
+    m->stats.partition_refused = background && ctx->part_refused ? 1 : 0;
     *inout = m;
     return rc;
 }
@@ -548,6 +686,40 @@
     return BEMB200_OK;
 }
 
+int bemb200_ctx_sm_partition(bemb200_ctx* ctx, int* sms) {
+    if (!ctx || !sms) return set_error(ctx, BEMB200_EINVAL, "NULL argument");
+    std::lock_guard<std::mutex> lk(ctx->mu);
+    BEMB_CUDA(ctx, cudaSetDevice(ctx->device));
+    *sms = ctx_ensure_partition(ctx);
+    return BEMB200_OK;
+}
+
+int bemb200_debug_partition_smids(bemb200_ctx* ctx, int* distinct) {
+    if (!ctx || !distinct) return set_error(ctx, BEMB200_EINVAL, "NULL argument");
+    std::lock_guard<std::mutex> lk(ctx->mu);
+    BEMB_CUDA(ctx, cudaSetDevice(ctx->device));
+    int sms = 0;
+    BEMB_CUDA(ctx, cudaDeviceGetAttribute(&sms, cudaDevAttrMultiProcessorCount, ctx->device));
+    const int part = ctx_ensure_partition(ctx);
+    cudaStream_t s = part ? ctx->part_stream : ctx->stream;
+    const unsigned int nb = 8u * (unsigned int)sms;
+    unsigned int* ids = nullptr;
+    BEMB_CUDA(ctx, cudaMalloc((void**)&ids, nb * sizeof(unsigned int)));
+    smid_kernel<<<nb, 128, 0, s>>>(ids);
+    cudaError_t e = cudaGetLastError();
+    std::vector<unsigned int> h(nb);
+    if (e == cudaSuccess) e = cudaMemcpyAsync(h.data(), ids, nb * sizeof(unsigned int), cudaMemcpyDeviceToHost, s);
+    if (e == cudaSuccess) e = cudaStreamSynchronize(s);
+    cudaFree(ids);
+    if (e != cudaSuccess) return cuda_fail(ctx, e, "smid_kernel");
+    std::vector<char> seen(1024, 0);
+    int n = 0;
+    for (unsigned int id : h)
+        if (id < seen.size() && !seen[id]) { seen[id] = 1; ++n; }
+    *distinct = n;
+    return BEMB200_OK;
+}
+
 int bemb200_ctx_set_shared_gpu(bemb200_ctx* ctx, int shared) {
     if (!ctx) return set_error(ctx, BEMB200_EINVAL, "NULL context");
     ctx->shared_gpu.store(shared ? 1 : 0);
diff --git a/math_audio_b200/csrc/api_internal.h b/math_audio_b200/csrc/api_internal.h
--- a/math_audio_b200/csrc/api_internal.h
+++ b/math_audio_b200/csrc/api_internal.h
@@ -63,6 +63,13 @@
     FusedLocal fx;
     std::shared_ptr<bemb::PeerGroup> group;
     int fused_grid = 0;
+    std::mutex part_mu;
+    bool part_tried = false;
+    bool part_refused = false;
+    int part_sms = 0;
+    void* part_green = nullptr;
+    cudaStream_t part_stream = nullptr;
+    cudaEvent_t part_join[2] = {nullptr, nullptr};
     std::string err;
     std::mutex mu;
 };
@@ -103,6 +110,7 @@
 int cuda_fail(bemb200_ctx* ctx, cudaError_t e, const char* what);
 void free_workspace(bemb200_matrix* m);
 void free_peer_exchange(bemb200_ctx* ctx, bool collective);
+int ctx_ensure_partition(bemb200_ctx* ctx);
 }
 
 #define BEMB_CUDA(ctx, call)                                          \
diff --git a/math_audio_b200/csrc/assembly_far.cu b/math_audio_b200/csrc/assembly_far.cu
--- a/math_audio_b200/csrc/assembly_far.cu
+++ b/math_audio_b200/csrc/assembly_far.cu
@@ -320,8 +320,8 @@
 
 template <int NQ, bool BIMAG, int MINB>
 cudaError_t launch_far_v(const DeviceMesh& m, const Phys& ph, uint64_t row_begin, uint64_t row_end, cplx* A, uint64_t lda,
-                         uint2* near_list, unsigned int near_cap, unsigned int* near_count, int background_blocks_per_sm,
-                         unsigned int* work_counter, FarRelaunch* relaunch, cudaStream_t s) {
+                         uint2* near_list, unsigned int near_cap, unsigned int* near_count, int background_sms,
+                         int background_blocks_per_sm, unsigned int* work_counter, FarRelaunch* relaunch, cudaStream_t s) {
     const uint64_t nrows = row_end - row_begin;
     uint32_t rpb = 128;
     while (rpb > 8 && (uint64_t)m.ntiles * ((nrows + rpb - 1) / rpb) < 148ull * MINB * 4ull) rpb >>= 1;
@@ -329,8 +329,9 @@
     const uint32_t total = m.ntiles * nchunks;
     uint32_t grid = total, ipb = 1;
     unsigned int* counter = nullptr;
-    if (background_blocks_per_sm > 0 && total > 148u * (uint32_t)background_blocks_per_sm) {
-        grid = 148u * (uint32_t)background_blocks_per_sm;
+    const uint32_t bg_grid = background_sms > 0 ? (uint32_t)background_sms * (uint32_t)(background_blocks_per_sm > 0 ? background_blocks_per_sm : MINB) : 0u;
+    if (bg_grid > 0 && total > bg_grid) {
+        grid = bg_grid;
         ipb = (total + grid - 1) / grid;
         grid = (total + ipb - 1) / ipb;
         counter = work_counter;
@@ -367,12 +368,12 @@
 
 template <int NQ>
 cudaError_t launch_far_t(const DeviceMesh& m, const Phys& ph, uint64_t row_begin, uint64_t row_end, cplx* A, uint64_t lda,
-                         uint2* near_list, unsigned int near_cap, unsigned int* near_count, int bg, unsigned int* work_counter,
-                         FarRelaunch* relaunch, cudaStream_t s) {
+                         uint2* near_list, unsigned int near_cap, unsigned int* near_count, int bg_sms, int bg,
+                         unsigned int* work_counter, FarRelaunch* relaunch, cudaStream_t s) {
     const bool bimag = (ph.beta.re == 0.0);
     static const int minb = env_int("BEMB200_FAR_MINB", 4);
 #define FAR_DISPATCH(B, M) \
-    return launch_far_v<NQ, B, M>(m, ph, row_begin, row_end, A, lda, near_list, near_cap, near_count, bg, work_counter, relaunch, s)
+    return launch_far_v<NQ, B, M>(m, ph, row_begin, row_end, A, lda, near_list, near_cap, near_count, bg_sms, bg, work_counter, relaunch, s)
     if (bimag) {
         if (minb == 2) FAR_DISPATCH(true, 2);
         if (minb == 3) FAR_DISPATCH(true, 3);
@@ -405,18 +406,18 @@
 int far_kernel_launch_count(const DeviceMesh& m) { return (m.n_flat_tri ? 1 : 0) + (m.n_flat_quad ? 1 : 0); }
 
 cudaError_t launch_far(const DeviceMesh& m, const Phys& ph, uint64_t row_begin, uint64_t row_end, cplx* A, uint64_t lda,
-                       uint2* near_list, unsigned int near_cap, unsigned int* near_count, int background_blocks_per_sm,
-                       unsigned int* work_counters, FarRelaunch* relaunch, cudaStream_t s) {
+                       uint2* near_list, unsigned int near_cap, unsigned int* near_count, int background_sms,
+                       int background_blocks_per_sm, unsigned int* work_counters, FarRelaunch* relaunch, cudaStream_t s) {
     if (row_end <= row_begin) return cudaSuccess;
     cudaError_t e = upload_tables();
     if (e != cudaSuccess) return e;
     if (m.n_flat_tri) {
-        e = launch_far_t<NQ_TRI>(m, ph, row_begin, row_end, A, lda, near_list, near_cap, near_count, background_blocks_per_sm,
+        e = launch_far_t<NQ_TRI>(m, ph, row_begin, row_end, A, lda, near_list, near_cap, near_count, background_sms, background_blocks_per_sm,
                                  work_counters ? work_counters + 0 : nullptr, relaunch, s);
         if (e != cudaSuccess) return e;
     }
     if (m.n_flat_quad) {
-        e = launch_far_t<NQ_QUAD>(m, ph, row_begin, row_end, A, lda, near_list, near_cap, near_count, background_blocks_per_sm,
+        e = launch_far_t<NQ_QUAD>(m, ph, row_begin, row_end, A, lda, near_list, near_cap, near_count, background_sms, background_blocks_per_sm,
                                   work_counters ? work_counters + 1 : nullptr, relaunch, s);
         if (e != cudaSuccess) return e;
     }
diff --git a/math_audio_b200/csrc/internal.h b/math_audio_b200/csrc/internal.h
--- a/math_audio_b200/csrc/internal.h
+++ b/math_audio_b200/csrc/internal.h
@@ -54,8 +54,8 @@
 cudaError_t launch_prep(const DeviceMesh& m, cudaStream_t s);
 typedef std::vector<std::function<cudaError_t(cudaStream_t)>> FarRelaunch;
 cudaError_t launch_far(const DeviceMesh& m, const Phys& ph, uint64_t row_begin, uint64_t row_end, cplx* A, uint64_t lda,
-                       uint2* near_list, unsigned int near_cap, unsigned int* near_count, int background_blocks_per_sm,
-                       unsigned int* work_counters, FarRelaunch* relaunch, cudaStream_t s);
+                       uint2* near_list, unsigned int near_cap, unsigned int* near_count, int background_sms,
+                       int background_blocks_per_sm, unsigned int* work_counters, FarRelaunch* relaunch, cudaStream_t s);
 cudaError_t launch_rhs_far(const DeviceMesh& m, const Phys& ph, uint64_t row_begin, uint64_t row_end, cplx* rhs, cudaStream_t s);
 cudaError_t launch_near_list(const DeviceMesh& m, const Phys& ph, uint64_t row_begin, cplx* A, uint64_t lda, cplx* rhs,
                              const uint2* near_list, unsigned int count, cudaStream_t s);
diff --git a/math_audio_b200/csrc/sweep.cu b/math_audio_b200/csrc/sweep.cu
--- a/math_audio_b200/csrc/sweep.cu
+++ b/math_audio_b200/csrc/sweep.cu
@@ -28,6 +28,7 @@
     bool buf_handed[2] = {false, false};
     uint64_t n = 0, r0 = 0, r1 = 0;
     bool overlap = true;
+    bool partitioned = false;
     int background = 1;
     std::thread worker;
     std::mutex mu;
@@ -93,6 +94,7 @@
     if (sw->overlap) {
         rc = bemb200_ctx_create_ex(device, rank, nranks, nullptr, nullptr, &sw->ctx_asm);
         if (rc != BEMB200_OK) { bemb200_ctx_destroy(sw->ctx_solve); return rc; }
+        sw->partitioned = ctx_ensure_partition(sw->ctx_asm) > 0;
     } else {
         sw->ctx_asm = sw->ctx_solve;
     }
@@ -151,7 +153,7 @@
             return set_error(sw->ctx_solve, job->rc, job->err);
         }
         sw->solving = true;
-        bemb200_ctx_set_shared_gpu(sw->ctx_solve, (sw->overlap && sw->queue.size() > 1) ? 1 : 0);
+        bemb200_ctx_set_shared_gpu(sw->ctx_solve, (sw->overlap && !sw->partitioned && sw->queue.size() > 1) ? 1 : 0);
     }
     bemb200_matrix* m = sw->buf[job->slot];
     int rc = BEMB200_OK;
diff --git a/math_audio_b200/sweep.py b/math_audio_b200/sweep.py
--- a/math_audio_b200/sweep.py
+++ b/math_audio_b200/sweep.py
@@ -140,7 +140,8 @@
         if err:
             raise err[0]
         self.ctx_asm.set_background(self.background_blocks_per_sm)
-        self.ctx_solve.set_shared_gpu(self.overlap)
+        shared = self.overlap and self.ctx_asm.sm_partition() == 0
+        self.ctx_solve.set_shared_gpu(shared)
         try:
             for i in range(len(cases)):
                 t = None
diff --git a/rust/bem-b200-sys/src/lib.rs b/rust/bem-b200-sys/src/lib.rs
--- a/rust/bem-b200-sys/src/lib.rs
+++ b/rust/bem-b200-sys/src/lib.rs
@@ -13,7 +13,8 @@
 #[repr(C)] pub struct bemb200_multi_matrix { _p: [u8; 0] }
 #[repr(C)] #[derive(Clone, Copy, Default)]
 pub struct bemb200_assembly_stats { pub near_pairs: u64, pub special_pairs: u64, pub far_kernel_launches: u64,
-                                    pub total_launches: u64, pub far_ms: f64, pub total_ms: f64 }
+                                    pub total_launches: u64, pub far_ms: f64, pub total_ms: f64,
+                                    pub partition_sms: i32, pub partition_refused: i32 }
 
 #[repr(C)]
 pub struct bemb200_mesh {
@@ -37,6 +38,7 @@
     pub fn bemb200_ctx_destroy(ctx: *mut bemb200_ctx);
     pub fn bemb200_ctx_set_background(ctx: *mut bemb200_ctx, blocks_per_sm: c_int) -> c_int;
     pub fn bemb200_ctx_set_shared_gpu(ctx: *mut bemb200_ctx, shared: c_int) -> c_int;
+    pub fn bemb200_ctx_sm_partition(ctx: *mut bemb200_ctx, sms: *mut c_int) -> c_int;
     pub fn bemb200_ctx_peer_exchange_active(ctx: *const bemb200_ctx, active: *mut c_int) -> c_int;
     pub fn bemb200_last_error(ctx: *const bemb200_ctx) -> *const c_char;
     pub fn bemb200_partition(n: u64, nranks: c_int, rank: c_int, row_begin: *mut u64, row_end: *mut u64);
```
